# stijnherfst/BrickMap

Hardware: AMD Instinct MI355X
Metric: Mrays/sec (primary x spp x bounces) at 1080p 4-bounce (higher is better)
Workload: dtype f32

## Files before the change

brickmap_amd/_lib.py:

```python
import ctypes as C
import os

_HERE = os.path.dirname(os.path.abspath(__file__))
LIB_PATH = os.path.join(_HERE, "libbrickmap_hip.so")

BM_FLAG_PRIMARY_ONLY = 1
BM_FLAG_SAMPLE_ITEMS = 4
BM_FLAG_COUNTERS = 2
BM_FLAG_ORDERED = 16
BM_FLAG_RAY_DIGEST = 32
BM_QUERY_LOD = 1
BM_QUERY_NO_REQUESTS = 2
BM_VOLUME_ANY = 1
BM_VOXELS_HOST = 0
BM_VOXELS_DEVICE = 1
BRICK_INDEX_BITS = 0x00000FFF
BRICK_LOD_BITS = 0x000FF000
BRICK_REQUESTED_BIT = 0x20000000
BRICK_UNLOADED_BIT = 0x40000000
BRICK_LOADED_BIT = 0x80000000


class BrickmapError(RuntimeError):
    pass
# ... 41 lines not shown

class bm_ray(C.Structure):
    _fields_ = [("origin", C.c_float * 3), ("direction", C.c_float * 3), ("tmax", C.c_float), ("reserved", C.c_uint32)]


class bm_ray_hit(C.Structure):
    _fields_ = [("distance", C.c_float), ("normal", C.c_float * 3), ("voxel", C.c_int32 * 3), ("level", C.c_int32)]


class bm_reproject_params(C.Structure):
    _fields_ = [("width", C.c_int32), ("height", C.c_int32), ("max_history", C.c_float), ("flags", C.c_uint32), ("reserved", C.c_uint32)]


class bm_denoise_params(C.Structure):
    _fields_ = [("width", C.c_int32), ("height", C.c_int32), ("iterations", C.c_int32), ("sigma_l", C.c_float), ("flags", C.c_uint32), ("reserved", C.c_uint32)]


class bm_volume(C.Structure):
    _fields_ = [("shape", C.c_int32), ("lo", C.c_int32 * 3), ("hi", C.c_int32 * 3), ("center", C.c_int32 * 3), ("radius", C.c_int32), ("reserved", C.c_uint32)]


class bm_volume_result(C.Structure):
    _fields_ = [("solid", C.c_uint64), ("lo", C.c_int32 * 3), ("hi", C.c_int32 * 3), ("unresolved", C.c_uint32), ("status", C.c_uint32)]


class bm_scene_info(C.Structure):
    _fields_ = [("grid_size", C.c_int32), ("grid_height", C.c_int32), ("supergrid_xy", C.c_int32),
                ("supergrid_z", C.c_int32), ("supercells", C.c_int32), ("queue_capacity", C.c_int32),
                ("lod_distance_8x8x8", C.c_int32), ("lod_distance_2x2x2", C.c_int32),
                ("generated", C.c_int32), ("on_device", C.c_int32),
                ("total_bricks", C.c_uint64), ("resident_bricks", C.c_uint64),
                ("index_bytes", C.c_uint64), ("brick_bytes", C.c_uint64),
                ("pool_bytes", C.c_uint64), ("cube_field_bytes", C.c_uint64),
                ("arena_growths", C.c_uint64), ("arena_copy_growths", C.c_uint64), ("arena_virtual", C.c_int32), ("failed", C.c_int32),
                ("stream_batches", C.c_uint64), ("stream_host_ns", C.c_uint64), ("escape_bytes", C.c_uint64), ("sun_plane_bytes", C.c_uint64)]


COUNTER_NAMES = ("index_loads", "brick_tests", "byte_tests", "voxel_steps", "extend_rays",
                 "shadow_rays", "requests", "paths")


class bm_counters(C.Structure):
    _fields_ = [(n, C.c_uint64) for n in COUNTER_NAMES]

    def as_dict(self):
        return {n: int(getattr(self, n)) for n in COUNTER_NAMES}


SCHED_NAMES = ("step_runs", "step_lanes", "candidate_runs", "candidate_lanes", "shade_runs", "shade_lanes", "connect_runs", "connect_lanes",
               "step_cycles", "candidate_cycles", "shade_cycles", "drain_cycles", "total_cycles", "jump_runs", "jump_lanes", "waves")


class bm_sched_stats(C.Structure):
    _fields_ = [(n, C.c_uint64) for n in SCHED_NAMES]


_vp, _i, _u32p = C.c_void_p, C.c_int, C.POINTER(C.c_uint32)
SIGNATURES = {
    "bm_last_error_string": (C.c_char_p, []),
    "bm_device_count": (_i, [C.POINTER(C.c_int)]),
    "bm_device_name": (_i, [_i, C.c_char_p, C.c_size_t, C.POINTER(C.c_int)]),
    "bm_scene_create": (_i, [_i, _i, _i, C.POINTER(_vp)]),
    "bm_scene_destroy": (None, [_vp]),
    "bm_scene_set_lod": (_i, [_vp, _i, _i]),
    "bm_scene_set_queue_capacity": (_i, [_vp, _i]),
    "bm_scene_set_streaming_mode": (_i, [_vp, _i]),
    "bm_scene_generate": (_i, [_vp, _i]),
    "bm_scene_generate_supercell": (_i, [_vp, _i, _i, _i]),
    "bm_scene_preload_all": (_i, [_vp]),
    "bm_scene_reset_residency": (_i, [_vp]),
    "bm_scene_process_load_queue": (_i, [_vp, _u32p]),
    "bm_scene_dump": (_i, [_vp, C.c_char_p]),
    "bm_scene_get_info": (_i, [_vp, C.POINTER(bm_scene_info)]),
    "bm_scene_host_supercell": (_i, [_vp, _i, _vp, _u32p, _vp, C.c_uint32]),
    "bm_scene_device_indices": (_i, [_vp, _i, _vp]),
    "bm_scene_device_brick": (_i, [_vp, _i, C.c_uint32, _vp]),
    "bm_scene_column_heights": (_i, [_vp, _i, _i, _vp]),
    "bm_scene_edit": (_i, [_vp, _i, C.POINTER(bm_edit), _vp]),
    "bm_scene_set_voxels": (_i, [_vp, _i, _vp, _vp, _vp]),
    "bm_scene_device_cube_field": (_i, [_vp, _vp, C.c_size_t, C.POINTER(C.c_size_t)]),
    "bm_scene_host_cube_field": (_i, [_vp, _vp, C.c_size_t, C.POINTER(C.c_size_t)]),
    "bm_scene_escape_table": (_i, [_vp, _vp, C.c_size_t, C.POINTER(C.c_size_t)]),
    "bm_scene_sun_plane": (_i, [_vp, _vp, C.c_size_t, C.POINTER(C.c_size_t), _vp]),
    "bm_scene_sun_plane_stats": (_i, [_vp, C.POINTER(C.c_uint64), C.POINTER(C.c_float)]),
    "bm_scene_last_edit_ms": (_i, [_vp, C.POINTER(C.c_float), C.POINTER(C.c_float)]),
    "bm_scene_load_voxels": (_i, [_vp, _vp, C.c_size_t, _i, _vp]),
    "bm_scene_host_voxels": (_i, [_vp, _vp, C.c_size_t, C.POINTER(C.c_size_t)]),
    "bm_scene_last_load_ms": (_i, [_vp, C.POINTER(C.c_float), C.POINTER(C.c_float), C.POINTER(C.c_float)]),
    "bm_scene_write_region": (_i, [_vp, C.POINTER(bm_region), _i, _vp, _i, _vp]),
    "bm_scene_read_region": (_i, [_vp, C.POINTER(bm_region), _vp, _i, _vp]),
    "bm_scene_last_region_ms": (_i, [_vp] + [C.POINTER(C.c_float)] * 4),
    "bm_scene_cast_rays": (_i, [_vp, C.c_int64, _vp, _vp, C.c_uint32, _vp, _vp]),
    "bm_scene_query_volumes": (_i, [_vp, C.c_int64, _vp, _vp, C.c_uint32, _vp]),
    "bm_camera_pixel_rays": (_i, [C.POINTER(bm_camera), _i, _i, C.c_int64, _vp, _vp, _vp]),
    "bm_camera_pixel_rays_device": (_i, [_vp, C.POINTER(bm_camera), _i, _i, _vp, _vp]),
    "bm_denoise_workspace_bytes": (_i, [_i, _i, C.POINTER(C.c_size_t)]),
    "bm_denoise": (_i, [_vp, C.POINTER(bm_denoise_params), _vp, _vp, _vp, _vp, C.c_size_t, _vp]),
    "bm_debug_denoise_times": (_i, [_vp, C.POINTER(bm_denoise_params), _vp, _vp, _vp, _vp, C.c_size_t, _vp, C.POINTER(C.c_float)]),
    "bm_host_denoise": (_i, [C.POINTER(bm_denoise_params), _vp, _vp, _vp]),
    "bm_history_bytes": (_i, [_i, _i, C.POINTER(C.c_size_t)]),
    "bm_reproject": (_i, [_vp, C.POINTER(bm_reproject_params), C.POINTER(bm_camera), C.POINTER(bm_camera), _vp, _vp, _vp, _vp, _vp]),
    "bm_host_reproject": (_i, [C.POINTER(bm_reproject_params), C.POINTER(bm_camera), C.POINTER(bm_camera), _vp, _vp, _vp, _vp]),
    "bm_host_column_heights": (_i, [_i, _i, _i, _i, _vp]),
    "bm_host_generate_supercell": (_i, [_i, _i, _i, _i, _i, _vp, _u32p, _vp, C.c_uint32]),
    "bm_host_edit_supercell": (_i, [_i, _i, _i, _i, _i, _vp, _u32p, _vp, C.c_uint32, _i, C.POINTER(bm_edit)]),
    "bm_host_write_region_supercell": (_i, [_i, _i, _i, _i, _i, _vp, _u32p, _vp, C.c_uint32, C.POINTER(bm_region), _i, _vp]),
    "bm_host_load_supercell": (_i, [_i, _i, _i, _i, _i, _vp, _vp, _vp, _u32p]),
    "bm_host_cube_field": (_i, [_i, _i, _vp, C.c_size_t, C.POINTER(C.c_size_t)]),
    "bm_buffer_alloc": (_i, [_i, C.c_size_t, C.POINTER(_vp)]),
    "bm_buffer_free": (_i, [_i, _vp]),
    "bm_buffer_zero": (_i, [_i, _vp, C.c_size_t, _vp]),
    "bm_buffer_read": (_i, [_i, _vp, _vp, C.c_size_t]),
    "bm_buffer_write": (_i, [_i, _vp, _vp, C.c_size_t]),
    "bm_local_rows": (_i, [C.POINTER(bm_frame_params)]),
    "bm_render_frame": (_i, [_vp, C.POINTER(bm_camera), C.POINTER(bm_frame_params), _vp, _vp, _vp]),
    "bm_render_frames": (_i, [_vp, _i, C.POINTER(bm_camera), C.POINTER(bm_frame_params), C.POINTER(_vp), C.POINTER(_vp), _vp]),
    "bm_frame_plan_of": (_i, [C.POINTER(bm_frame_params), _i, C.POINTER(bm_frame_plan)]),
    "bm_launch_plan_of": (_i, [_i, C.POINTER(bm_camera), C.POINTER(bm_frame_params), _vp, _vp, _i, _i, C.POINTER(bm_launch_plan)]),
    "bm_trace_waves_per_simd": (_i, [_i, _i, _i, _i, C.POINTER(C.c_int)]),
    "bm_tuning_overrides": (_i, [C.c_char_p, C.c_size_t]),
    "bm_resolve": (_i, [_vp, _vp, _vp, C.c_int64, _vp]),
    "bm_synchronize": (_i, [_vp]),
    "bm_last_render_ms": (_i, [_vp, C.POINTER(C.c_float)]),
    "bm_render_times": (_i, [_vp, _vp, _i, C.POINTER(C.c_int)]),
    "bm_counters_read": (_i, [_vp, C.POINTER(bm_counters)]),
    "bm_counters_reset": (_i, [_vp]),
    "bm_sched_stats_read": (_i, [_vp, C.POINTER(bm_sched_stats)]),
    "bm_sched_detail_read": (_i, [_vp, _vp]),
    "bm_wavefront_create": (_i, [_vp, C.c_uint32, C.POINTER(_vp)]),
    "bm_wavefront_destroy": (None, [_vp]),
    "bm_wavefront_reset": (_i, [_vp]),
    "bm_wavefront_frame": (_i, [_vp, C.POINTER(bm_camera), C.POINTER(bm_frame_params), _vp, _vp]),
    "bm_wavefront_stats": (_i, [_vp, _u32p]),
    "bm_wavefront_read_queue": (_i, [_vp, _i, C.c_uint32, C.c_uint32, _vp]),
    "bm_wavefront_times": (_i, [_vp, C.POINTER(C.c_float)]),
    "bm_wavefront_counters_read": (_i, [_vp, _i, C.POINTER(bm_counters)]),
    "bm_wavefront_counters_reset": (_i, [_vp]),
    "bm_wavefront_sched_stats_read": (_i, [_vp, _i, C.POINTER(C.c_uint64)]),
    "bm_comm_unique_id": (_i, [_vp]),
    "bm_comm_create": (_i, [_i, _i, _i, _vp, C.POINTER(_vp)]),
    "bm_comm_destroy": (None, [_vp]),
    "bm_comm_info": (_i, [_vp, C.POINTER(C.c_int), C.POINTER(C.c_int)]),
    "bm_comm_available": (_i, []),
    "bm_debug_division_magic": (_i, [C.c_uint32, C.POINTER(C.c_uint32), C.POINTER(C.c_int)]),
    "bm_gather_frame": (_i, [_vp, _vp, _vp, _i, _i, _i, _i, _vp]),
    "bm_gather_frames": (_i, [_vp, _vp, _vp, _i, _i, _i, _i, _i, _vp]),
    "bm_reduce_frame": (_i, [_vp, _vp, _vp, C.c_int64, _i, _vp]),
    "bm_probe_streams": (_i, [_i, _i, C.POINTER(_vp)]),
    "bm_release_streams": (None, [_i, C.POINTER(_vp)]),
    "bm_comm_barrier": (_i, [_vp, _vp]),
    "bm_comm_selftest": (_i, [_vp, _vp]),
    "bm_debug_assemble_frame": (_i, [_i, _vp, _vp, _vp, _i, _i, _i, _i, _i, _i, _vp]),
    "bm_debug_sincos": (_i, [_i, _i, _vp, _vp, _vp]),
    "bm_debug_sky": (_i, [_i, _vp, _i, _vp, _vp, _vp, _vp]),
}

_lib = None


def load():
    global _lib
    if _lib is not None:
        return _lib
    if not os.path.exists(LIB_PATH):
        raise BrickmapError(
            f"{LIB_PATH} is missing: build it with `python -c 'import __graft_entry__ as g; g.build()'` "
# ... 19 lines not shown
```

brickmap_amd/csrc/capi.cpp:

```cpp
#include <cmath>
#include <cstdint>
#include <cstring>
#include <limits>
#include <string>
#include <vector>
#include <new>

#include "camera_rays.h"
#include "denoise.h"
#include "kernels.h"
#include "reproject.h"
#include "scene.h"
#include "wavefront.h"

struct bm_scene {
	bm::Scene impl;
	explicit bm_scene(int device) : impl(device) {}
};

struct bm_wavefront {
	bm::Wavefront impl;
	bm_wavefront(bm::Scene* scene, uint32_t queue_size) : impl(scene, queue_size) {}
};

// ... 21 lines not shown

int bm_device_name(int device, char* buf, size_t buflen, int* compute_units) {
	hipDeviceProp_t prop;
	BM_HIP(hipGetDeviceProperties(&prop, device));
	if (buf && buflen) {
		std::strncpy(buf, prop.gcnArchName, buflen - 1);
		buf[buflen - 1] = 0;
	}
	if (compute_units) *compute_units = prop.multiProcessorCount;
	return 0;
}

int bm_scene_create(int device, int grid_size, int grid_height, bm_scene** out) {
	if (!out) { set_error("null argument"); return BM_EINVAL; }
	*out = nullptr;
	bm_scene* s = new (std::nothrow) bm_scene(device);
	if (!s) { set_error("out of host memory"); return BM_EINVAL; }
	if (int e = s->impl.init(grid_size, grid_height)) {
		delete s;
		return e;
	}
	*out = s;
	return 0;
}

void bm_scene_destroy(bm_scene* scene) { delete scene; }

int bm_scene_set_lod(bm_scene* scene, int lod8, int lod2) { BM_NEED(scene); return scene->impl.set_lod(lod8, lod2); }
int bm_scene_set_queue_capacity(bm_scene* scene, int capacity) { BM_NEED(scene); return scene->impl.set_queue_capacity(capacity); }
int bm_scene_set_streaming_mode(bm_scene* scene, int overlapped) { BM_NEED(scene); return scene->impl.set_streaming_mode(overlapped); }
int bm_scene_generate(bm_scene* scene, int threads) { BM_NEED(scene); return scene->impl.generate(threads); }
int bm_scene_generate_supercell(bm_scene* scene, int sx, int sy, int sz) { BM_NEED(scene); return scene->impl.generate_supercell(sx, sy, sz); }
int bm_scene_preload_all(bm_scene* scene) { BM_NEED(scene); return scene->impl.preload_all(); }
int bm_scene_reset_residency(bm_scene* scene) { BM_NEED(scene); return scene->impl.reset_residency(); }
int bm_scene_process_load_queue(bm_scene* scene, uint32_t* serviced) { BM_NEED(scene); return scene->impl.process_load_queue(serviced); }
int bm_scene_dump(bm_scene* scene, const char* path) { BM_NEED(scene); return scene->impl.dump(path); }
int bm_scene_get_info(bm_scene* scene, bm_scene_info* info) { BM_NEED(scene); return scene->impl.info(info); }

int bm_scene_host_supercell(bm_scene* scene, int supercell, uint32_t* indices4096, uint32_t* brick_count, uint32_t* bricks, uint32_t brick_capacity) {
	BM_NEED(scene);
	bm::World& w = scene->impl.world;
	if (supercell < 0 || supercell >= static_cast<int>(w.supercells.size())) { set_error("bad supercell (or world not generated)"); return BM_EINVAL; }
	const bm::HostSupercell& c = w.supercells[supercell];
	if (c.indices.size() != static_cast<size_t>(bm::kCellsPerSupercell)) { set_error("supercell not generated"); return BM_ESTATE; }
	if (indices4096) std::memcpy(indices4096, c.indices.data(), bm::kCellsPerSupercell * sizeof(uint32_t));
	if (brick_count) *brick_count = static_cast<uint32_t>(c.bricks.size());
	if (bricks) {
		const size_t n = c.bricks.size() < brick_capacity ? c.bricks.size() : brick_capacity;
		std::memcpy(bricks, c.bricks.data(), n * sizeof(bm::Brick));
	}
	return 0;
}

int bm_scene_device_indices(bm_scene* scene, int supercell, uint32_t* indices4096) { BM_NEED(scene); return scene->impl.device_indices(supercell, indices4096); }

int bm_scene_device_brick(bm_scene* scene, int supercell, uint32_t device_slot, uint32_t* out16) { BM_NEED(scene); return scene->impl.device_brick(supercell, device_slot, out16); }

int bm_scene_edit(bm_scene* scene, int count, const bm_edit* edits, void* hip_stream) {
	BM_NEED(scene);
	return scene->impl.edit(count, edits, static_cast<hipStream_t>(hip_stream));
}

int bm_scene_set_voxels(bm_scene* scene, int n, const int32_t* xyz, const uint8_t* values, void* hip_stream) {
	BM_NEED(scene);
	if (n < 0 || (n > 0 && (!xyz || !values))) { set_error("bm_scene_set_voxels: bad count or null argument"); return BM_EINVAL; }
	std::vector<bm_edit> edits;
	edits.reserve(static_cast<size_t>(n));
	for (int i = 0; i < n; ++i) {
		const int32_t* v = xyz + 3 * static_cast<size_t>(i);
		if (v[0] < 0 || v[1] < 0 || v[2] < 0 || v[0] == INT32_MAX || v[1] == INT32_MAX || v[2] == INT32_MAX) continue;
		bm_edit e{};
		e.op = values[i] ? BM_EDIT_SET : BM_EDIT_CLEAR;
		e.shape = BM_EDIT_BOX;
		for (int k = 0; k < 3; ++k) { e.lo[k] = v[k]; e.hi[k] = v[k] + 1; }
		edits.push_back(e);
	}
	return scene->impl.edit(static_cast<int>(edits.size()), edits.data(), static_cast<hipStream_t>(hip_stream));
}

int bm_scene_device_cube_field(bm_scene* scene, uint8_t* dst, size_t capacity, size_t* bytes) { BM_NEED(scene); return scene->impl.device_cube_field(dst, capacity, bytes); }
int bm_scene_host_cube_field(bm_scene* scene, uint8_t* dst, size_t capacity, size_t* bytes) { BM_NEED(scene); return scene->impl.host_cube_field(dst, capacity, bytes); }
int bm_scene_escape_table(bm_scene* scene, int32_t* dst, size_t capacity, size_t* count) { BM_NEED(scene); return scene->impl.escape_table(dst, capacity, count); }
int bm_scene_sun_plane(bm_scene* scene, uint8_t* dst, size_t capacity, size_t* bytes, int32_t* plan12) { BM_NEED(scene); return scene->impl.sun_plane(dst, capacity, bytes, plan12); }
int bm_scene_sun_plane_stats(bm_scene* scene, uint64_t* builds, float* last_build_ms) { BM_NEED(scene); return scene->impl.sun_plane_stats(builds, last_build_ms); }
int bm_scene_last_edit_ms(bm_scene* scene, float* scatter_ms, float* field_ms) { BM_NEED(scene); return scene->impl.last_edit_ms(scatter_ms, field_ms); }

int bm_scene_load_voxels(bm_scene* scene, const uint8_t* voxels, size_t bytes, int where, void* hip_stream) {
	BM_NEED(scene);
	return scene->impl.load_voxels(voxels, bytes, where, static_cast<hipStream_t>(hip_stream));
}
int bm_scene_host_voxels(bm_scene* scene, uint8_t* dst, size_t capacity, size_t* bytes) { BM_NEED(scene); return scene->impl.host_voxels(dst, capacity, bytes); }
int bm_scene_last_load_ms(bm_scene* scene, float* pack_ms, float* field_ms, float* mirror_ms) { BM_NEED(scene); return scene->impl.last_load_ms(pack_ms, field_ms, mirror_ms); }

int bm_scene_write_region(bm_scene* scene, const bm_region* region, int op, const uint8_t* voxels, int where, void* hip_stream) {
	BM_NEED(scene);
	return scene->impl.write_region(region, op, voxels, where, static_cast<hipStream_t>(hip_stream));
}
int bm_scene_read_region(bm_scene* scene, const bm_region* region, uint8_t* voxels, int where, void* hip_stream) {
	BM_NEED(scene);
	return scene->impl.read_region(region, voxels, where, static_cast<hipStream_t>(hip_stream));
}
int bm_scene_last_region_ms(bm_scene* scene, float* pack_ms, float* copy_ms, float* scatter_ms, float* field_ms) {
	BM_NEED(scene);
	return scene->impl.last_region_ms(pack_ms, copy_ms, scatter_ms, field_ms);
}

int bm_scene_cast_rays(bm_scene* scene, int64_t n, const bm_ray* rays_dev, bm_ray_hit* hits_dev, uint32_t flags, const float lod_origin[3], void* hip_stream) {
	BM_NEED(scene);
	return scene->impl.cast_rays(n, rays_dev, hits_dev, flags, lod_origin, static_cast<hipStream_t>(hip_stream));
}

int bm_scene_query_volumes(bm_scene* scene, int64_t n, const bm_volume* volumes_dev, bm_volume_result* results_dev, uint32_t flags, void* hip_stream) {
	BM_NEED(scene);
	return scene->impl.query_volumes(n, volumes_dev, results_dev, flags, static_cast<hipStream_t>(hip_stream));
}

int bm_camera_pixel_rays(const bm_camera* camera, int width, int height, int64_t n, const float* px, const float* py, bm_ray* out) {
	if (!camera || width <= 0 || height <= 0 || width > 65535 || height > 65535 || n < 0 || (n > 0 && (!px || !py || !out))) {
		set_error("bm_camera_pixel_rays: bad argument");
		return BM_EINVAL;
	}
	bm_frame_params p{};
	p.width = width; p.height = height; p.spp = 1; p.band_rows = height; p.shard_count = 1;
	bm::FrameConstants fc;
	if (int e = bm::fill_frame_constants(camera, &p, &fc)) return e;
	const float W = static_cast<float>(width), H = static_cast<float>(height);
	for (int64_t i = 0; i < n; ++i) {
		bm_ray& r = out[i];
		bm::pixel_ray_direction(fc.dir, fc.right, fc.up, W, H, px[i], py[i], r.direction);
		for (int k = 0; k < 3; ++k) r.origin[k] = fc.origin[k];
		r.tmax = std::numeric_limits<float>::infinity();
		r.reserved = 0;
	}
	return 0;
}

int bm_camera_pixel_rays_device(bm_scene* scene, const bm_camera* camera, int width, int height, bm_ray* rays_dev, void* hip_stream) {
	BM_NEED(scene);
	return scene->impl.pixel_rays(camera, width, height, rays_dev, static_cast<hipStream_t>(hip_stream));
}

int bm_denoise_workspace_bytes(int width, int height, size_t* bytes) {
	if (!bytes || width < 1 || height < 1 || width > 65535 || height > 65535) { set_error("bm_denoise_workspace_bytes: bad argument"); return BM_EINVAL; }
	*bytes = bm::denoise_workspace_bytes(width, height);
	return 0;
}

int bm_denoise(bm_scene* scene, const bm_denoise_params* params, const float* accum_dev, const bm_ray_hit* hits_dev, float* out_dev, void* workspace_dev,
			   size_t workspace_bytes, void* hip_stream) {
	BM_NEED(scene);
	return scene->impl.denoise(params, accum_dev, hits_dev, out_dev, workspace_dev, workspace_bytes, static_cast<hipStream_t>(hip_stream));
}

int bm_debug_denoise_times(bm_scene* scene, const bm_denoise_params* params, const float* accum_dev, const bm_ray_hit* hits_dev, float* out_dev,
						   void* workspace_dev, size_t workspace_bytes, void* hip_stream, float* kernel_ms) {
	BM_NEED(scene);
	if (!kernel_ms) { set_error("bm_debug_denoise_times: null argument"); return BM_EINVAL; }
	return scene->impl.denoise(params, accum_dev, hits_dev, out_dev, workspace_dev, workspace_bytes, static_cast<hipStream_t>(hip_stream), kernel_ms);
}

int bm_history_bytes(int width, int height, size_t* bytes) {
	if (!bytes || width < 1 || height < 1 || width > 65535 || height > 65535) { set_error("bm_history_bytes: bad argument"); return BM_EINVAL; }
	*bytes = bm::history_bytes(width, height);
	return 0;
}

// ... 354 lines not shown
```

brickmap_amd/csrc/kernels.h:

```cpp
#pragma once
#include <hip/hip_runtime.h>

#include "device_types.h"
#include "reproject.h"
#include "sunfield.h"

namespace bm {
template <class K>
int resident_blocks_per_cu(K kernel, int threads = 256) {
	int n = 0;
	const hipError_t e = hipOccupancyMaxActiveBlocksPerMultiprocessor(&n, kernel, threads, 0);
	return e == hipSuccess && n > 0 ? n : 1;
}

constexpr size_t kWorkCounterBytes = 64 * 32 * sizeof(uint32_t);
int trace_blocks_per_cu(bool instrumented, bool xcd_handout, bool helpers, int ring = 0);
void launch_trace(const DeviceScene& sc, const FrameConstants* fc_dev, DeviceCounters* counters, uint32_t* work_counter, bool instrumented, bool xcd_handout, bool helpers,
				  int ring, long long workgroups, int compute_units, int blocks_per_cu_cap, hipStream_t stream);
void launch_upload(const DeviceScene& sc, const uint32_t* bricks_queue, const uint32_t* indices_queue, uint32_t* arena, uint32_t count,
				   hipStream_t stream);
void launch_pool_moves(const PoolMove* moves, uint32_t count, uint32_t* arena, uint32_t* pool_base, hipStream_t stream);
void launch_snapshot_ring(const int* queue, const uint32_t* count, int* host_positions, uint32_t* host_count, uint32_t capacity, hipStream_t stream);
void launch_resolve(const float* accum, float* out, long long n, hipStream_t stream);
void launch_debug_sincos(int n, const float* x, float* s, float* c, hipStream_t stream);
void launch_debug_sky(const FrameConstants& fc, int n, const float* v, float* sun, float* sky, float* sunsky, hipStream_t stream);

struct FieldUpdate {
	int rx0, rx1, ry0, ry1, rz0, rz1;
	int ay0, ay1, bz0, bz1;
	int cells, cells_height, sg_xy, sg_xy2;
	int cf_shift;
	uint32_t cf_pxy, cf_plane;
};
size_t field_update_tmp_bytes(const FieldUpdate& u);
void launch_edit_scatter(const uint32_t* cells, const uint32_t* words, const uint32_t* slots, const uint32_t* bricks, uint32_t count,
						 uint32_t* index_grid, uint32_t* arena, hipStream_t stream);
void launch_field_update(const uint32_t* index_grid, uint8_t* field, uint8_t* tmp, const FieldUpdate& u, hipStream_t stream);

struct EscapeUpdate {
	int x0, x1, y0, y1;
	int cells, cells_height, sg_xy, sg_xy2;
	int cf_shift;
	uint32_t cf_pxy, cf_plane;
};
size_t escape_columns_bytes(int cells);
void launch_escape_update(const uint32_t* index_grid, int32_t* cols, uint32_t* table, const EscapeUpdate& u, hipStream_t stream);

struct SunBuild {
	SunPlan plan;
	int cells, cells_height, sg_xy, sg_xy2;
	int nd, n1, n2;
	int cf_shift;
	uint32_t cf_pxy, cf_plane;
};
size_t sun_build_tmp_bytes(const SunBuild& u);
void launch_sun_build(const uint32_t* index_grid, const int32_t* cols, const uint32_t* escape, uint8_t* field, uint8_t* tmp, const SunBuild& u, hipStream_t stream);

struct LoadDims {
	uint32_t grid_size;
	uint32_t sg_xy, sg_xy2;
	uint32_t supercells;
};
void launch_load_classify(const uint8_t* voxels, uint32_t* index_grid, const LoadDims& d, hipStream_t stream);
void launch_load_number(uint32_t* index_grid, uint32_t* counts, uint32_t* pool_base, uint32_t* total, const LoadDims& d, hipStream_t stream);
void launch_load_pack(const uint8_t* voxels, const uint32_t* index_grid, const uint32_t* pool_base, uint32_t* arena, const LoadDims& d, hipStream_t stream);

struct RegionDims {
	int lo[3], hi[3], org[3];
	int c0[3], nc[3], g0;
	uint32_t sg_xy, sg_xy2;
	int64_t row_pitch, slice_pitch;
};
void launch_region_pack(const uint8_t* voxels, uint32_t* bricks, const RegionDims& d, hipStream_t stream);
void launch_region_unpack(uint8_t* voxels, const uint32_t* index_grid, const uint32_t* pool_base, const uint32_t* arena, const RegionDims& d, hipStream_t stream);
void launch_region_patch(uint8_t* voxels, const int* cells, const uint32_t* bricks, uint32_t count, const RegionDims& d, hipStream_t stream);
void launch_region_zero(uint8_t* voxels, int64_t row_pitch, int64_t slice_pitch, int64_t nx, int64_t ny, int64_t nz, hipStream_t stream);

int query_blocks_per_cu(bool request);
void launch_query(const DeviceScene& sc, const int campos[3], const void* rays, void* hits, uint32_t n, uint32_t* ticket, int resident_blocks,
				  bool request, hipStream_t stream);

int volume_blocks_per_cu(bool any);
size_t volume_tmp_bytes(uint32_t n);
void launch_volume_query(const DeviceScene& sc, const void* volumes, void* results, uint32_t n, bool any, uint64_t* tmp, int resident_blocks, hipStream_t stream);

constexpr int kDenoiseTiledMaxStep = 2;
void launch_denoise(int width, int height, int iterations, float sigma_l, const float* accum, const void* hits, float* out, void* workspace,
					int tiled_max_step, hipStream_t stream, hipEvent_t* marks = nullptr);
struct PixelRayBasis {
	float right[3], up[3], dir[3], origin[3];
	int width, height;
};
void launch_pixel_rays(const PixelRayBasis& basis, void* rays, hipStream_t stream);
struct ReprojectCameras {
	CameraBasis cur;
	RpPrevCamera prev;
	int width, height;
};
void launch_reproject(const ReprojectCameras& cams, float max_history, const float* accum, const void* hits, const void* history_prev, void* history_out,
					  hipStream_t stream);

int wavefront_blocks_per_cu(bool connect, bool instrumented);
void launch_wf_primary(WfState* st, WfRay* work, const FrameConstants* fc_dev, uint32_t queue_size, uint32_t pixels, hipStream_t stream);
void launch_wf_trace(bool connect, const DeviceScene& sc, const FrameConstants* fc_dev, WfState* st, WfRay* work, const WfShadow* shadow, float* accum,
					 DeviceCounters* counters, uint32_t queue_size, int resident_blocks, void* cold_scratch, hipStream_t stream);
void launch_wf_shade(const WfRay* work, WfRay* next, WfShadow* shadow, float* accum, void* block_counts, WfState* st, const FrameConstants* fc_dev,
					 uint32_t queue_size, hipStream_t stream);
}
```

brickmap_amd/csrc/scene.cpp:

```cpp
#include "scene.h"

#include <algorithm>
#include <atomic>
#include <chrono>
#include <climits>
#include <cmath>
#include <cstddef>
#include <cstdio>
#include <cstdlib>
#include <cstring>
#include <fstream>
#include <thread>
#include <unordered_map>

#include "camera_rays.h"
#include "denoise.h"
#include "escape.h"
#include "kernels.h"

namespace bm {

static thread_local std::string g_error;
void set_error(const std::string& msg) { g_error = msg; }
const char* last_error() { return g_error.c_str(); }
// ... 49 lines not shown
	if (!on_device_) { set_error("scene not generated"); return BM_ESTATE; }
	return 0;
}

int Scene::require_not_failed() const {
	if (failed_) { set_error("a streaming batch failed on this scene: call bm_scene_reset_residency / bm_scene_preload_all"); return BM_ESTATE; }
	return 0;
}

int Scene::init(int grid_size, int grid_height) {
	if (!world.dims.set(grid_size, grid_height)) {
		set_error("grid_size and grid_height must be positive multiples of 128 voxels");
		return BM_EINVAL;
	}
	if (world.dims.cells > 1024 || world.dims.cells_height > 1024) {
		set_error("world too large: at most 8192 voxels along an axis (and see the cube-field limit: cubic worlds up to 5760 voxels a side)");
		return BM_EINVAL;
	}
	if (!cube_field_layout(world.dims).fits) {
		set_error("world too large: the octant cube field (8 planes of (cells_h + 2) x (cells + 2) rows padded to a power of two) must stay below 4 GiB -- cubic worlds up to 5760 voxels a side");
		return BM_EINVAL;
	}
	BM_HIP(hipSetDevice(device_));
	if (int e = load_stream_.create(hipStreamNonBlocking)) return e;
	if (int e = kernel_stream_.create(hipStreamNonBlocking)) return e;
	for (int i = 0; i < kTimingRing; ++i) {
		if (int e = ev_start_[i].create()) return e;
		if (int e = ev_stop_[i].create()) return e;
	}
	for (Event* ev : {&ev_upload_, &ev_snapshot_, &ev_edit_, &ev_edit_caller_}) if (int e = ev->create(hipEventDisableTiming)) return e;
	for (Event& ev : ev_edit_time_) if (int e = ev.create()) return e;
	for (int r = 0; r < 2; ++r) {
		if (int e = h_count_[r].alloc(sizeof(uint32_t))) return e;
		if (int e = d_load_count_[r].alloc(sizeof(uint32_t))) return e;
		BM_HIP(hipMemset(d_load_count_[r], 0, sizeof(uint32_t)));
	}
	if (int e = d_counters_.alloc(sizeof(DeviceCounters))) return e;
	BM_HIP(hipMemset(d_counters_, 0, sizeof(DeviceCounters)));
	if (int e = d_work_counter_.alloc(kWorkCounterBytes * kFrameRing)) return e;
	if (int e = d_frame_constants_.alloc(kFrameRing * sizeof(FrameConstants))) return e;
	if (int e = h_frame_constants_.alloc(kFrameRing * sizeof(FrameConstants))) return e;
	std::fill(ring_owner_, ring_owner_ + kFrameRing, -1ll);
	hipDeviceProp_t prop;
	BM_HIP(hipGetDeviceProperties(&prop, device_));
	compute_units_ = prop.multiProcessorCount;
	blocks_per_cu_[0] = blocks_per_cu_[1] = 0;
	if (tuning().blocks_per_cu > 0) blocks_per_cu_[0] = tuning().blocks_per_cu;

	return alloc_queue();
}

int Scene::alloc_queue() {
	BM_HIP(hipSetDevice(device_));
	const size_t n = static_cast<size_t>(queue_cap_);
	for (int r = 0; r < 2; ++r) {
		if (int e = h_positions_[r].alloc(n * 3 * sizeof(int))) return e;
		if (int e = d_load_queue_[r].alloc(n * 3 * sizeof(int))) return e;
		BM_HIP(hipMemset(d_load_queue_[r], 0, n * 3 * sizeof(int)));
		BM_HIP(hipMemset(d_load_count_[r], 0, sizeof(uint32_t)));
	}
	if (int e = h_bricks_.alloc(n * sizeof(Brick))) return e;
	if (int e = h_indices_.alloc(n * sizeof(uint32_t))) return e;
	if (int e = d_bricks_queue_.alloc(n * sizeof(Brick))) return e;
	if (int e = d_indices_queue_.alloc(n * sizeof(uint32_t))) return e;
	if (int e = d_positions_.alloc(n * 3 * sizeof(int))) return e;
	if (int e = h_moves_.alloc(n * sizeof(PoolMove))) return e;
	if (int e = d_moves_.alloc(n * sizeof(PoolMove))) return e;
	use_ring(0);
	snapshot_pending_ = false;
	view_.queue_cap = static_cast<uint32_t>(queue_cap_);
	return 0;
}

void Scene::use_ring(int ring) {
	ring_cur_ = ring;
	view_.load_queue = d_load_queue_[ring];
	view_.load_queue_count = d_load_count_[ring];
}

void Scene::residency_rebuilt(bool preloaded) {
	use_ring(0);
	snapshot_pending_ = false;
	preloaded_ = preloaded;
	staging_busy_ = false;
	failed_ = false;
	stream_batches_ = stream_host_ns_ = 0;
	upload_seq_ = 0;
	for (FrameStream& f : frame_streams_) f.upload_seen = 0;
}

int Scene::set_streaming_mode(int overlapped) {
	BM_HIP(hipSetDevice(device_));
	BM_HIP(hipDeviceSynchronize());
	if (snapshot_pending_) {
		snapshot_pending_ = false;
		const uint32_t count = std::min<uint32_t>(static_cast<uint32_t>(queue_cap_), *h_count_[ring_snapshot_]);
		if (count > 0) {
			if (int e = service_ring(ring_snapshot_, count, nullptr)) return e;
		}
		BM_HIP(hipDeviceSynchronize());
	}
	if (overlapped_ && !overlapped && ring_cur_ != 0) {
		BM_HIP(hipMemcpy(d_load_queue_[0], d_load_queue_[1], static_cast<size_t>(queue_cap_) * 3 * sizeof(int), hipMemcpyDeviceToDevice));
		BM_HIP(hipMemcpy(d_load_count_[0], d_load_count_[1], sizeof(uint32_t), hipMemcpyDeviceToDevice));
		BM_HIP(hipMemset(d_load_count_[1], 0, sizeof(uint32_t)));
		use_ring(0);
	}
	overlapped_ = overlapped != 0;
	return 0;
}

int Scene::set_lod(int lod8, int lod2) {
	lod8_ = lod8;
	lod2_ = lod2;
	view_.lod_distance_8x8x8 = lod8;
	view_.lod_distance_2x2x2 = lod2;
	return 0;
}

int Scene::set_queue_capacity(int cap) {
	if (cap <= 0) { set_error("queue capacity must be positive"); return BM_EINVAL; }
	if (on_device_) { set_error("set the queue capacity before bm_scene_generate"); return BM_ESTATE; }
	BM_HIP(hipSetDevice(device_));
	BM_HIP(hipDeviceSynchronize());
	queue_cap_ = cap;
	return alloc_queue();
}

void Scene::free_device() {
	(void)d_index_grid_.release();
	(void)d_pool_base_.release();
	arena_.close();
	(void)d_cube_field_.release();
	sun_plane_ = sun_built_ = false;
	(void)d_escape_.release();
	(void)d_escape_cols_.release();
	on_device_ = false;
}

int Scene::arena_fit(uint64_t bricks) {
	arena_.reset();
	bool left_unmapped = false;
	const int e = arena_.reserve(std::max<uint64_t>(bricks, 1), true, &left_unmapped);
	if (left_unmapped) failed_ = true;
	view_.brick_arena = arena_.base();
	return e;
}

int Scene::pool_region(uint32_t bricks, uint32_t* offset) {
	const int e = arena_.region_alloc(bricks, offset);
	view_.brick_arena = arena_.base();
	return e;
}

int Scene::allocate_device() {
	BM_HIP(hipSetDevice(device_));
	free_device();
	const WorldDims& d = world.dims;
	uint64_t run = 0;
	for (int i = 0; i < d.supercells; ++i) run += world.supercells[i].bricks.size();
	if (run >= (1ull << 32)) { set_error("world has more than 2^32 bricks"); return BM_EINVAL; }
	if (int e = alloc_index_grid()) return e;
	if (int e = arena_.open(device_, 4 * run + 32ull * static_cast<uint64_t>(d.supercells) + (1ull << 16))) return e;
	view_.brick_arena = arena_.base();
	if (int e = alloc_cube_field()) return e;
	{
		std::vector<uint8_t> field;
		world.build_cube_field(field, 8);
		const int X = d.cells + 2, Z = d.cells_height + 2;
		for (int o = 0; o < 8; ++o)
			BM_HIP(hipMemcpy2D(d_cube_field_ + static_cast<size_t>(o) * view_.cf_plane, static_cast<size_t>(1) << view_.cf_shift, field.data() + static_cast<size_t>(o) * X * X * Z, X, X,
							   static_cast<size_t>(X) * Z, hipMemcpyHostToDevice));
	}
	set_view_dims();
	on_device_ = true;
	if (int e = reset_residency()) return e;
	launch_escape_update(d_index_grid_, d_escape_cols_, d_escape_, escape_update_box(0, d.cells, 0, d.cells), load_stream_);
	BM_HIP(hipGetLastError());
	BM_HIP(hipStreamSynchronize(load_stream_));
	return 0;
}

int Scene::alloc_index_grid() {
	const WorldDims& d = world.dims;
	const size_t index_bytes = static_cast<size_t>(d.supercells) * kCellsPerSupercell * sizeof(uint32_t);
	if (int e = d_index_grid_.alloc(index_bytes)) return e;
	if (int e = d_pool_base_.alloc(static_cast<size_t>(d.supercells) * sizeof(uint32_t))) return e;
	BM_HIP(hipMemset(d_pool_base_, 0, static_cast<size_t>(d.supercells) * sizeof(uint32_t)));
	view_.index_grid = d_index_grid_;
	view_.pool_base = d_pool_base_;
	view_.brick_arena = nullptr;
	return 0;
}

int Scene::alloc_cube_field() {
	const CubeFieldLayout l = cube_field_layout(world.dims);
	if (!l.fits) { set_error("world too large for the 32-bit cube-field offsets of the walk"); return BM_EINVAL; }
	sun_plane_ = false;
	if (l.ninth) {
		if (d_cube_field_.alloc(l.plane * 9) == 0) sun_plane_ = true;
		else { (void)hipGetLastError(); set_error(""); }
	}
	if (!sun_plane_) { if (int e = d_cube_field_.alloc(l.plane * 8)) return e; }
	sun_built_ = false;
	sun_dirty_ = true;
	BM_HIP(hipMemset(d_cube_field_, 255, d_cube_field_.bytes()));
	view_.cf_shift = l.shift;
	view_.cf_pxy = static_cast<uint32_t>(l.pxy);
	view_.cf_plane = static_cast<uint32_t>(l.plane);
	division_magic(view_.cf_pxy, &view_.cf_magic, &view_.cf_magic_shift);
	view_.cube_field = d_cube_field_;
	if (int e = d_escape_.alloc(escape_entries(view_.cf_pxy) * sizeof(uint32_t))) return e;
	BM_HIP(hipMemset(d_escape_, 0, d_escape_.bytes()));
	if (int e = d_escape_cols_.alloc(escape_columns_bytes(world.dims.cells))) return e;
	view_.escape = d_escape_;
	return 0;
}

EscapeUpdate Scene::escape_update_box(int x0, int x1, int y0, int y1) const {
	const WorldDims& d = world.dims;
	EscapeUpdate u{};
	u.x0 = std::max(0, x0); u.x1 = std::min(d.cells, x1); u.y0 = std::max(0, y0); u.y1 = std::min(d.cells, y1);
	if (u.x1 < u.x0) u.x1 = u.x0;
	if (u.y1 < u.y0) u.y1 = u.y0;
	u.cells = d.cells; u.cells_height = d.cells_height;
	u.sg_xy = d.supergrid_xy; u.sg_xy2 = d.supergrid_xy * d.supergrid_xy;
	u.cf_shift = view_.cf_shift; u.cf_pxy = view_.cf_pxy; u.cf_plane = view_.cf_plane;
	return u;
}

void Scene::set_view_dims() {
	const WorldDims& d = world.dims;
	view_.cells = d.cells;
	view_.cells_height = d.cells_height;
	view_.sg_xy = d.supergrid_xy;
	view_.sg_xy2 = d.supergrid_xy * d.supergrid_xy;
	view_.grid_size_f = static_cast<float>(d.grid_size);
	view_.grid_height_f = static_cast<float>(d.grid_height);
	view_.lod_distance_8x8x8 = lod8_;
	view_.lod_distance_2x2x2 = lod2_;
}

int Scene::generate(int threads) {
	world.generate(threads);
	return allocate_device();
}

int Scene::generate_supercell(int sx, int sy, int sz) {
	const WorldDims& d = world.dims;
	if (sx < 0 || sy < 0 || sz < 0 || sx >= d.supergrid_xy || sy >= d.supergrid_xy || sz >= d.supergrid_z) {
		set_error("supercell coordinates out of range");
		return BM_EINVAL;
	}
	if (on_device_) { set_error("bm_scene_generate_supercell: the scene is on the device (call it before bm_scene_generate)"); return BM_ESTATE; }
	world.generate_supercell(sx, sy, sz);
	return 0;
}

int Scene::reset_residency() {
	if (int e = require_on_device()) return e;
	BM_HIP(hipSetDevice(device_));
	BM_HIP(hipDeviceSynchronize());
	const WorldDims& d = world.dims;
	std::vector<uint32_t> words(static_cast<size_t>(d.supercells) * kCellsPerSupercell);
	std::vector<uint32_t> bases(d.supercells, 0u);
	uint64_t initial = 0;
	for (int i = 0; i < d.supercells; ++i) initial += world.supercells[i].bricks.empty() ? 0u : kStartingPool;
	if (int e = arena_fit(initial)) return e;
	for (int i = 0; i < d.supercells; ++i) {
		HostSupercell& c = world.supercells[i];
		c.resident = 0;
		c.pool_capacity = 0;
		c.pool_base = 0;
		c.dev_slot.assign(c.bricks.size(), kNoDeviceSlot);
		c.pool_free.clear();
		if (!c.bricks.empty()) {
			if (int e = pool_region(kStartingPool, &c.pool_base)) return e;
			c.pool_capacity = kStartingPool;
		}
		bases[i] = c.pool_base;
		uint32_t* dst = &words[static_cast<size_t>(i) * kCellsPerSupercell];
		for (int j = 0; j < kCellsPerSupercell; ++j)
			dst[j] = (c.indices[j] & BM_BRICK_LOADED_BIT) ? (BM_BRICK_UNLOADED_BIT | (c.indices[j] & BM_BRICK_LOD_BITS)) : 0u;
	}
	BM_HIP(hipMemcpy(d_index_grid_, words.data(), words.size() * sizeof(uint32_t), hipMemcpyHostToDevice));
	BM_HIP(hipMemcpy(d_pool_base_, bases.data(), bases.size() * sizeof(uint32_t), hipMemcpyHostToDevice));
	for (int r = 0; r < 2; ++r) BM_HIP(hipMemset(d_load_count_[r], 0, sizeof(uint32_t)));
	resident_bricks_ = 0;
	residency_rebuilt(false);
	return 0;
}

int Scene::preload_all() {
	if (int e = require_on_device()) return e;
	BM_HIP(hipSetDevice(device_));
// ... 297 lines not shown
			launch_pool_moves(d_moves_, n_moves, arena_.base(), d_pool_base_, load_stream_);
			BM_HIP(hipGetLastError());
		}
		launch_upload(ring_view, d_bricks_queue_, d_indices_queue_, arena_.base(), kept, load_stream_);
		BM_HIP(hipGetLastError());
		BM_HIP(hipMemsetAsync(d_load_count_[ring], 0, sizeof(uint32_t), load_stream_));
		BM_HIP(hipEventRecord(ev_upload_, load_stream_));
		return 0;
	};
	if (int e = queue()) { failed_ = true; return e; }
	arena_.commit_freed_regions();
	staging_busy_ = true;
	upload_seq_++;
	resident_bricks_ += kept;
	if (serviced) *serviced = kept;
	stream_batches_++;
	stream_host_ns_ += static_cast<uint64_t>(std::chrono::duration_cast<std::chrono::nanoseconds>(std::chrono::steady_clock::now() - t_host0).count());
	return 0;
}

int Scene::process_load_queue(uint32_t* serviced) {
	if (serviced) *serviced = 0;
	if (int e = require_on_device()) return e;
	if (int e = require_not_failed()) return e;
	BM_HIP(hipSetDevice(device_));
	if (!overlapped_) {
		if (int e = wait_frames_on_host()) return e;
		BM_HIP(hipMemcpyAsync(h_count_[0], d_load_count_[0], sizeof(uint32_t), hipMemcpyDeviceToHost, load_stream_));
		BM_HIP(hipStreamSynchronize(load_stream_));
		const uint32_t count = std::min<uint32_t>(static_cast<uint32_t>(queue_cap_), *h_count_[0]);
		if (count == 0) return 0;
		BM_HIP(hipMemcpyAsync(h_positions_[0], d_load_queue_[0], static_cast<size_t>(count) * 3 * sizeof(int), hipMemcpyDeviceToHost, load_stream_));
		BM_HIP(hipStreamSynchronize(load_stream_));
		return service_ring(0, count, serviced);
	}
	if (snapshot_pending_) {
		BM_HIP(hipEventSynchronize(ev_snapshot_));
		snapshot_pending_ = false;
		const uint32_t count = std::min<uint32_t>(static_cast<uint32_t>(queue_cap_), *h_count_[ring_snapshot_]);
		if (count > 0) {
			if (int e = service_ring(ring_snapshot_, count, serviced)) return e;
		}
	}
	if (int e = order_load_stream_behind_frames()) return e;
	const int ring = ring_cur_;
	{
		int* dev_positions = nullptr;
		uint32_t* dev_count = nullptr;
		BM_HIP(hipHostGetDevicePointer(reinterpret_cast<void**>(&dev_positions), h_positions_[ring], 0));
		BM_HIP(hipHostGetDevicePointer(reinterpret_cast<void**>(&dev_count), h_count_[ring], 0));
		launch_snapshot_ring(d_load_queue_[ring], d_load_count_[ring], dev_positions, dev_count, static_cast<uint32_t>(queue_cap_), load_stream_);
		BM_HIP(hipGetLastError());
	}
	BM_HIP(hipEventRecord(ev_snapshot_, load_stream_));
	snapshot_pending_ = true;
	ring_snapshot_ = ring;
	use_ring(ring ^ 1);
	return 0;
}

int Scene::dump(const char* path) {
	std::ofstream file(path ? path : "dump.txt");
	if (!file) { set_error("cannot open dump file"); return BM_EINVAL; }
	for (const auto& c : world.supercells) file << c.resident << "\n";
	return 0;
}

int Scene::info(bm_scene_info* out) {
	if (!out) { set_error("null argument"); return BM_EINVAL; }
	const WorldDims& d = world.dims;
	std::memset(out, 0, sizeof *out);
	out->grid_size = d.grid_size; out->grid_height = d.grid_height;
	out->supergrid_xy = d.supergrid_xy; out->supergrid_z = d.supergrid_z; out->supercells = d.supercells;
	out->queue_capacity = queue_cap_;
	out->lod_distance_8x8x8 = lod8_; out->lod_distance_2x2x2 = lod2_;
	out->generated = world.generated ? 1 : 0;
	out->on_device = on_device_ ? 1 : 0;
	out->total_bricks = world.generated ? world.total_bricks() : 0;
	out->resident_bricks = resident_bricks_;
	out->index_bytes = on_device_ ? static_cast<uint64_t>(d.supercells) * kCellsPerSupercell * 4 : 0;
	out->brick_bytes = on_device_ ? arena_.capacity() * 64 : 0;
	out->pool_bytes = on_device_ ? arena_.pool_bricks() * 64 : 0;
	out->cube_field_bytes = on_device_ ? 8 * static_cast<uint64_t>(view_.cf_plane) : 0;
	out->escape_bytes = on_device_ ? d_escape_.bytes() : 0;
	out->sun_plane_bytes = on_device_ && sun_plane_ ? static_cast<uint64_t>(view_.cf_plane) + d_sun_tmp_.bytes() : 0;
	out->arena_growths = arena_.growths();
	out->arena_copy_growths = arena_.copy_growths();
	out->arena_virtual = arena_.is_virtual() ? 1 : 0;
	out->failed = failed_ ? 1 : 0;
	out->stream_batches = stream_batches_;
	out->stream_host_ns = stream_host_ns_;
	return 0;
}

int Scene::device_indices(int supercell, uint32_t* out4096) {
	if (int e = require_on_device()) return e;
	if (supercell < 0 || supercell >= world.dims.supercells || !out4096) { set_error("bad supercell"); return BM_EINVAL; }
	BM_HIP(hipSetDevice(device_));
	BM_HIP(hipDeviceSynchronize());
	BM_HIP(hipMemcpy(out4096, d_index_grid_ + static_cast<size_t>(supercell) * kCellsPerSupercell, kCellsPerSupercell * 4, hipMemcpyDeviceToHost));
	return 0;
}

int Scene::device_brick(int supercell, uint32_t device_slot, uint32_t* out16) {
	if (int e = require_on_device()) return e;
	if (supercell < 0 || supercell >= world.dims.supercells || !out16 || device_slot >= world.supercells[supercell].resident) {
		set_error("bad supercell or slot");
		return BM_EINVAL;
	}
	BM_HIP(hipSetDevice(device_));
	BM_HIP(hipDeviceSynchronize());
	BM_HIP(hipMemcpy(out16, arena_.base() + (static_cast<size_t>(world.supercells[supercell].pool_base) + device_slot) * kBrickWords, sizeof(Brick), hipMemcpyDeviceToHost));
	return 0;
}

int Scene::edit(int count, const bm_edit* edits, hipStream_t stream) {
	std::string why;
	if (!World::validate_edits(edits, count, &why)) { set_error("bm_scene_edit: " + why); return BM_EINVAL; }
	if (!on_device_) { set_error("bm_scene_edit: scene not generated"); return BM_ESTATE; }
	if (int e = require_not_failed()) return e;
	const WorldDims& d = world.dims;
	std::vector<int> reached;
	{
		std::vector<uint8_t> seen(static_cast<size_t>(d.supercells), 0);
		for (int i = 0; i < count; ++i) {
			int lo[3], hi[3];
			if (!World::edit_bounds(d, edits[i], lo, hi)) continue;
			for (int sz = lo[2] / kColumnSpan; sz <= (hi[2] - 1) / kColumnSpan; ++sz)
				for (int sy = lo[1] / kColumnSpan; sy <= (hi[1] - 1) / kColumnSpan; ++sy)
					for (int sx = lo[0] / kColumnSpan; sx <= (hi[0] - 1) / kColumnSpan; ++sx) {
						const int sc = d.supercell_id(sx, sy, sz);
						if (!seen[sc]) { seen[sc] = 1; reached.push_back(sc); }
					}
		}
	}
	if (reached.empty()) return 0;
	std::sort(reached.begin(), reached.end());
	BM_HIP(hipSetDevice(device_));
	if (int e = wait_edit_staging()) return e;

	DeviceBatch batch;
	std::vector<uint32_t> old_words;
	std::vector<uint8_t> touched;
	for (const int sci : reached) {
		HostSupercell& c = world.supercells[sci];
		const int sx = sci % d.supergrid_xy, sy = (sci / d.supergrid_xy) % d.supergrid_xy, sz = sci / (d.supergrid_xy * d.supergrid_xy);
		old_words = c.indices;
		touched.assign(kCellsPerSupercell, 0);
		World::edit_supercell(d, c, sx, sy, sz, edits, count, touched.data());
		if (int e = stage_touched(sci, old_words, touched.data(), batch)) return e;
	}
	bool scattered = false, field = false;
	if (int e = submit_batch(batch, stream, ev_edit_time_, &scattered, &field)) return e;
	if (scattered) {
		edit_timed_ = true;
		edit_field_timed_ = field;
	}
	return 0;
}

int Scene::wait_edit_staging() {
	if (edit_busy_) { BM_HIP(hipEventSynchronize(ev_edit_)); edit_busy_ = false; }
	return 0;
}

int Scene::stage_touched(int sci, const std::vector<uint32_t>& old_words, const uint8_t* touched, DeviceBatch& b) {
	const WorldDims& d = world.dims;
	HostSupercell& c = world.supercells[sci];
	const int sx = sci % d.supergrid_xy, sy = (sci / d.supergrid_xy) % d.supergrid_xy, sz = sci / (d.supergrid_xy * d.supergrid_xy);
	const std::vector<uint16_t>& old_dev = c.dev_slot;
	std::vector<uint16_t> dev(c.bricks.size(), kNoDeviceSlot);
	for (int j = 0; j < kCellsPerSupercell; ++j)
		if (c.indices[j] && !touched[j]) dev[c.indices[j] & BM_BRICK_INDEX_BITS] = old_dev[c.indices[j] & BM_BRICK_INDEX_BITS];
	std::vector<int> fresh_cells;
	for (int j = 0; j < kCellsPerSupercell; ++j) {
		if (!touched[j]) continue;
		const uint32_t ow = old_words[j], nw = c.indices[j];
		const uint16_t ods = ow ? old_dev[ow & BM_BRICK_INDEX_BITS] : kNoDeviceSlot;
		if (ods != kNoDeviceSlot) {
			if (nw) dev[nw & BM_BRICK_INDEX_BITS] = ods;
			else { c.pool_free.push_back(ods); resident_bricks_--; }
		} else if (nw && preloaded_) {
			fresh_cells.push_back(j);
		}
		if ((ow != 0) != (nw != 0)) {
			const int g[3] = {sx * kSupercell + (j & 15), sy * kSupercell + ((j >> 4) & 15), sz * kSupercell + (j >> 8)};
			for (int k = 0; k < 3; ++k) { b.box_lo[k] = std::min(b.box_lo[k], g[k]); b.box_hi[k] = std::max(b.box_hi[k], g[k]); }
		}
	}
	if (!fresh_cells.empty()) {
		const uint32_t reuse = static_cast<uint32_t>(std::min(fresh_cells.size(), c.pool_free.size()));
		const uint32_t appends = static_cast<uint32_t>(fresh_cells.size()) - reuse;
		if (c.resident + appends > c.pool_capacity) {
			uint32_t grown = kStartingPool;
			while (grown < c.resident + appends || grown < 2 * c.pool_capacity) grown *= 2;
			uint32_t fresh = 0;
			if (int e = pool_region(grown, &fresh)) { failed_ = true; return e; }
			b.moves.push_back(PoolMove{c.pool_capacity ? c.pool_base : fresh, fresh, c.pool_capacity ? c.resident : 0u, static_cast<uint32_t>(sci)});
			if (c.pool_capacity > 0) arena_.region_free_deferred(c.pool_capacity, c.pool_base);
			c.pool_base = fresh;
			c.pool_capacity = grown;
		}
		for (const int j : fresh_cells) {
			uint32_t ds;
			if (!c.pool_free.empty()) { ds = c.pool_free.back(); c.pool_free.pop_back(); }
			else ds = c.resident++;
			dev[c.indices[j] & BM_BRICK_INDEX_BITS] = static_cast<uint16_t>(ds);
			resident_bricks_++;
		}
	}
	c.dev_slot.swap(dev);
	for (int j = 0; j < kCellsPerSupercell; ++j) {
		if (!touched[j]) continue;
		const uint32_t nw = c.indices[j];
		const uint16_t ds = nw ? c.dev_slot[nw & BM_BRICK_INDEX_BITS] : kNoDeviceSlot;
		b.cells.push_back(static_cast<uint32_t>(sci) * kCellsPerSupercell + static_cast<uint32_t>(j));
		if (!nw) b.words.push_back(0u);
		else if (ds == kNoDeviceSlot) b.words.push_back(BM_BRICK_UNLOADED_BIT | (nw & BM_BRICK_LOD_BITS));
		else b.words.push_back(ds | BM_BRICK_LOADED_BIT | (nw & BM_BRICK_LOD_BITS));
		b.slots.push_back(ds == kNoDeviceSlot ? 0xFFFFFFFFu : c.pool_base + ds);
		b.bricks.push_back(nw ? c.bricks[nw & BM_BRICK_INDEX_BITS] : Brick{});
	}
	return 0;
}

int Scene::submit_batch(DeviceBatch& b, hipStream_t stream, Event* times, bool* scattered, bool* field_updated) {
	const WorldDims& d = world.dims;
	*scattered = *field_updated = false;
	const uint32_t n = static_cast<uint32_t>(b.cells.size());
	if (n == 0) {
		arena_.commit_freed_regions();
		return 0;
	}

	auto up = [](size_t v) { return (v + 63) / 64 * 64; };
	const size_t o_cells = up(b.moves.size() * sizeof(PoolMove)), o_words = o_cells + up(n * 4ull), o_slots = o_words + up(n * 4ull),
				 o_bricks = o_slots + up(n * 4ull), bytes = o_bricks + n * sizeof(Brick);
	const bool field = b.box_hi[0] >= 0;
	const FieldUpdate fu = field ? field_update_box(d, b.box_lo, b.box_hi) : FieldUpdate{};
	auto queue = [&]() -> int {
		if (bytes > d_edit_.bytes()) {
			BM_HIP(hipStreamSynchronize(load_stream_));
			const size_t cap = std::max<size_t>(bytes * 2, 1 << 16);
			if (int e = h_edit_.reserve(cap)) return e;
			if (int e = d_edit_.reserve(cap)) return e;
		}
		if (field && field_update_tmp_bytes(fu) > d_cf_tmp_.bytes()) {
			BM_HIP(hipStreamSynchronize(load_stream_));
			if (int e = d_cf_tmp_.reserve(field_update_tmp_bytes(fu))) return e;
		}
		if (!b.moves.empty()) std::memcpy(h_edit_, b.moves.data(), b.moves.size() * sizeof(PoolMove));
		std::memcpy(h_edit_ + o_cells, b.cells.data(), n * 4ull);
		std::memcpy(h_edit_ + o_words, b.words.data(), n * 4ull);
		std::memcpy(h_edit_ + o_slots, b.slots.data(), n * 4ull);
		std::memcpy(h_edit_ + o_bricks, b.bricks.data(), n * sizeof(Brick));
		if (int e = order_load_stream_behind_frames()) return e;
		BM_HIP(hipEventRecord(ev_edit_caller_, stream));
		BM_HIP(hipStreamWaitEvent(load_stream_, ev_edit_caller_, 0));
		BM_HIP(hipMemcpyAsync(d_edit_, h_edit_, bytes, hipMemcpyHostToDevice, load_stream_));
		BM_HIP(hipEventRecord(ev_edit_, load_stream_));
		BM_HIP(hipEventRecord(times[0], load_stream_));
		if (!b.moves.empty()) {
			launch_pool_moves(reinterpret_cast<const PoolMove*>(d_edit_.get()), static_cast<uint32_t>(b.moves.size()), arena_.base(), d_pool_base_, load_stream_);
			BM_HIP(hipGetLastError());
		}
		launch_edit_scatter(reinterpret_cast<const uint32_t*>(d_edit_ + o_cells), reinterpret_cast<const uint32_t*>(d_edit_ + o_words),
							reinterpret_cast<const uint32_t*>(d_edit_ + o_slots), reinterpret_cast<const uint32_t*>(d_edit_ + o_bricks), n, d_index_grid_, arena_.base(),
							load_stream_);
		BM_HIP(hipGetLastError());
		BM_HIP(hipEventRecord(times[1], load_stream_));
		if (field) {
			launch_field_update(d_index_grid_, d_cube_field_, d_cf_tmp_, fu, load_stream_);
			BM_HIP(hipGetLastError());
			launch_escape_update(d_index_grid_, d_escape_cols_, d_escape_, escape_update_box(b.box_lo[0], b.box_hi[0] + 1, b.box_lo[1], b.box_hi[1] + 1), load_stream_);
			BM_HIP(hipGetLastError());
			sun_dirty_ = true;
		}
		BM_HIP(hipEventRecord(times[2], load_stream_));
		BM_HIP(hipEventRecord(ev_upload_, load_stream_));
		return 0;
	};
	if (int e = queue()) { failed_ = true; return e; }
	arena_.commit_freed_regions();
	edit_busy_ = true;
	upload_seq_++;
	*scattered = true;
	*field_updated = field;
	return 0;
}

int Scene::last_edit_ms(float* scatter_ms, float* field_ms) {
	if (!scatter_ms || !field_ms) { set_error("null argument"); return BM_EINVAL; }
	if (!edit_timed_) { set_error("no edit has changed the scene yet"); return BM_ESTATE; }
	BM_HIP(hipSetDevice(device_));
	BM_HIP(hipEventSynchronize(ev_edit_time_[2]));
	BM_HIP(hipEventElapsedTime(scatter_ms, ev_edit_time_[0], ev_edit_time_[1]));
	BM_HIP(hipEventElapsedTime(field_ms, ev_edit_time_[1], ev_edit_time_[2]));
	if (!edit_field_timed_) *field_ms = 0.0f;
	return 0;
}

namespace {
template <class F> void for_outside_slabs(const int32_t blo[3], const int32_t bhi[3], bool inside, const int lo[3], const int hi[3], F f) {
	if (!inside) { f(blo[0], bhi[0], blo[1], bhi[1], blo[2], bhi[2]); return; }
	if (blo[2] < lo[2]) f(blo[0], bhi[0], blo[1], bhi[1], blo[2], lo[2]);
	if (hi[2] < bhi[2]) f(blo[0], bhi[0], blo[1], bhi[1], hi[2], bhi[2]);
	if (blo[1] < lo[1]) f(blo[0], bhi[0], blo[1], lo[1], lo[2], hi[2]);
	if (hi[1] < bhi[1]) f(blo[0], bhi[0], hi[1], bhi[1], lo[2], hi[2]);
	if (blo[0] < lo[0]) f(blo[0], lo[0], lo[1], hi[1], lo[2], hi[2]);
	if (hi[0] < bhi[0]) f(hi[0], bhi[0], lo[1], hi[1], lo[2], hi[2]);
}
int64_t region_offset(const bm_region& r, int64_t x, int64_t y, int64_t z) { return (z - r.lo[2]) * r.slice_pitch + (y - r.lo[1]) * r.row_pitch + (x - r.lo[0]); }
}

int Scene::check_region(const char* who, const bm_region* region, const void* voxels, int where, bm_region* r, uint64_t* span) {
	const std::string at = std::string(who) + ": ";
	if (!region || !voxels) { set_error(at + "null region or volume"); return BM_EINVAL; }
	*r = *region;
	std::string why;
	if (!World::validate_region(r, &why, span)) { set_error(at + why); return BM_EINVAL; }
	if (where != BM_VOXELS_HOST && where != BM_VOXELS_DEVICE) { set_error(at + "`where` is BM_VOXELS_HOST or BM_VOXELS_DEVICE"); return BM_EINVAL; }
	if (!on_device_) { set_error(at + "scene not generated"); return BM_ESTATE; }
	if (int e = require_not_failed()) return e;
	BM_HIP(hipSetDevice(device_));
	if (where == BM_VOXELS_DEVICE && *span > 0 && !device_span_ok(static_cast<const uint8_t*>(voxels), *span)) {
		set_error(at + "BM_VOXELS_DEVICE needs the volume's whole span inside one allocation of the scene's device");
		return BM_EINVAL;
	}
	return 0;
}

RegionDims Scene::region_dims(const bm_region& r, const int lo[3], const int hi[3]) const {
	RegionDims rd{};
	for (int k = 0; k < 3; ++k) {
		rd.lo[k] = lo[k]; rd.hi[k] = hi[k]; rd.org[k] = r.lo[k];
		rd.c0[k] = lo[k] >> 3;
		rd.nc[k] = ((hi[k] - 1) >> 3) - rd.c0[k] + 1;
	}
	rd.g0 = rd.c0[0] >> 4;
	rd.sg_xy = static_cast<uint32_t>(world.dims.supergrid_xy);
	rd.sg_xy2 = rd.sg_xy * rd.sg_xy;
	rd.row_pitch = r.row_pitch;
	rd.slice_pitch = r.slice_pitch;
	return rd;
}

int Scene::write_region(const bm_region* region, int op, const uint8_t* voxels, int where, hipStream_t stream) {
	bm_region r;
	uint64_t span = 0;
	if (op != BM_REGION_REPLACE && op != BM_EDIT_SET && op != BM_EDIT_CLEAR) { set_error("bm_scene_write_region: unknown op"); return BM_EINVAL; }
	if (int e = check_region("bm_scene_write_region", region, voxels, where, &r, &span)) return e;
	const WorldDims& d = world.dims;
	int lo[3], hi[3];
// ... 89 lines not shown
		});
		if (inside) world.store_region(lo, hi, r.lo, voxels, r.row_pitch, r.slice_pitch, 16);
		return 0;
	}
	std::vector<int> cells;
	std::vector<Brick> bricks;
	if (inside && !preloaded_)
		for (int cz = lo[2] >> 3; cz <= (hi[2] - 1) >> 3; ++cz)
			for (int cy = lo[1] >> 3; cy <= (hi[1] - 1) >> 3; ++cy)
				for (int cx = lo[0] >> 3; cx <= (hi[0] - 1) >> 3; ++cx) {
					const HostSupercell& c = world.supercells[d.supercell_id(cx / kSupercell, cy / kSupercell, cz / kSupercell)];
					const uint32_t word = c.indices[cell_local_index(cx, cy, cz)];
					if (word == 0 || c.dev_slot[word & BM_BRICK_INDEX_BITS] != kNoDeviceSlot) continue;
					cells.insert(cells.end(), {cx, cy, cz});
					bricks.push_back(c.bricks[word & BM_BRICK_INDEX_BITS]);
				}
	const size_t n = bricks.size(), o_bricks = (n * 3 * sizeof(int) + 63) / 64 * 64, bytes = o_bricks + n * sizeof(Brick);
	if (n > 0) {
		if (int e = ev_region_read_.create(hipEventDisableTiming)) return e;
		if (region_read_busy_) { BM_HIP(hipEventSynchronize(ev_region_read_)); region_read_busy_ = false; }
		if (int e = h_patch_.reserve(std::max<size_t>(bytes, 1 << 16))) return e;
		if (int e = d_patch_.reserve(std::max<size_t>(bytes, 1 << 16))) return e;
		std::memcpy(h_patch_, cells.data(), n * 3 * sizeof(int));
		std::memcpy(h_patch_ + o_bricks, bricks.data(), n * sizeof(Brick));
	}
	DeviceScene view;
	if (int e = begin_frame(stream, &view, nullptr)) return e;
	for_outside_slabs(r.lo, r.hi, inside, lo, hi, [&](int64_t x0, int64_t x1, int64_t y0, int64_t y1, int64_t z0, int64_t z1) {
		launch_region_zero(voxels + region_offset(r, x0, y0, z0), r.row_pitch, r.slice_pitch, x1 - x0, y1 - y0, z1 - z0, stream);
	});
	if (inside) {
		const RegionDims rd = region_dims(r, lo, hi);
		launch_region_unpack(voxels, view.index_grid, view.pool_base, view.brick_arena, rd, stream);
		if (n > 0) {
			BM_HIP(hipMemcpyAsync(d_patch_, h_patch_, bytes, hipMemcpyHostToDevice, stream));
			launch_region_patch(voxels, reinterpret_cast<const int*>(d_patch_.get()), reinterpret_cast<const uint32_t*>(d_patch_ + o_bricks), static_cast<uint32_t>(n), rd, stream);
			BM_HIP(hipEventRecord(ev_region_read_, stream));
			region_read_busy_ = true;
		}
	}
	BM_HIP(hipGetLastError());
	end_frame(stream);
	return 0;
}

int Scene::device_cube_field(uint8_t* dst, size_t capacity, size_t* bytes) {
	if (int e = require_on_device()) return e;
	const WorldDims& d = world.dims;
	const size_t X = static_cast<size_t>(d.cells) + 2, Z = static_cast<size_t>(d.cells_height) + 2, need = 8 * X * X * Z;
	if (bytes) *bytes = need;
	if (!dst) return 0;
	if (capacity < need) { set_error("cube field buffer too small"); return BM_EINVAL; }
	BM_HIP(hipSetDevice(device_));
	BM_HIP(hipDeviceSynchronize());
	BM_HIP(hipMemcpy2D(dst, X, d_cube_field_, static_cast<size_t>(1) << view_.cf_shift, X, 8 * X * Z, hipMemcpyDeviceToHost));
	return 0;
}

int Scene::escape_table(int32_t* dst, size_t capacity, size_t* count) {
	if (int e = require_on_device()) return e;
	const WorldDims& d = world.dims;
	const size_t plane = static_cast<size_t>(d.cells) * d.cells, need = 8 * plane;
	if (count) *count = need;
	if (!dst) return 0;
	if (capacity < need) { set_error("escape table buffer too small"); return BM_EINVAL; }
	BM_HIP(hipSetDevice(device_));
	BM_HIP(hipDeviceSynchronize());
	std::vector<uint32_t> entries(escape_entries(view_.cf_pxy));
	BM_HIP(hipMemcpy(entries.data(), d_escape_, entries.size() * sizeof(uint32_t), hipMemcpyDeviceToHost));
	for (int o = 0; o < 8; ++o)
		for (int y = 0; y < d.cells; ++y)
			for (int x = 0; x < d.cells; ++x)
				dst[o * plane + static_cast<size_t>(y) * d.cells + x] = escape_height_of(o, entries[escape_index(o, view_.cf_shift, view_.cf_pxy, x, y)], view_.cf_pxy, view_.cf_plane);
	return 0;
}

int Scene::ensure_sun_plane(const FrameConstants& fc, bool* usable) {
	*usable = false;
	if (!sun_plane_) return 0;
	const SunPlan plan = sun_plan(fc.cone_dir, fc.cone_extent);
	if (!plan.valid) return 0;
	const float key[4] = {fc.cone_dir[0], fc.cone_dir[1], fc.cone_dir[2], fc.cone_extent};
	*usable = true;
	if (sun_built_ && !sun_dirty_ && std::memcmp(key, sun_key_, sizeof key) == 0) return 0;
	const WorldDims& d = world.dims;
	const int n[3] = {d.cells, d.cells, d.cells_height};
	SunBuild u{};
	u.plan = plan;
	u.cells = d.cells; u.cells_height = d.cells_height;
	u.sg_xy = d.supergrid_xy; u.sg_xy2 = d.supergrid_xy * d.supergrid_xy;
	u.nd = n[plan.dom]; u.n1 = n[plan.m1]; u.n2 = n[plan.m2];
	u.cf_shift = view_.cf_shift; u.cf_pxy = view_.cf_pxy; u.cf_plane = view_.cf_plane;
	*usable = false;
	for (Event& ev : ev_sun_time_) if (int e = ev.create()) return e;
	if (sun_build_tmp_bytes(u) > d_sun_tmp_.bytes()) {
		BM_HIP(hipStreamSynchronize(load_stream_));
		if (d_sun_tmp_.reserve(sun_build_tmp_bytes(u)) != 0) { (void)hipGetLastError(); set_error(""); return 0; }
	}
	if (int e = order_load_stream_behind_frames()) return e;
	BM_HIP(hipEventRecord(ev_sun_time_[0], load_stream_));
	launch_sun_build(d_index_grid_, d_escape_cols_, d_escape_, d_cube_field_, d_sun_tmp_, u, load_stream_);
	BM_HIP(hipGetLastError());
	BM_HIP(hipEventRecord(ev_sun_time_[1], load_stream_));
	BM_HIP(hipEventRecord(ev_upload_, load_stream_));
	upload_seq_++;
	std::memcpy(sun_key_, key, sizeof key);
	sun_plan_ = plan;
	sun_built_ = true;
	sun_dirty_ = false;
	sun_builds_++;
	*usable = true;
	return 0;
}

int Scene::sun_plane(uint8_t* dst, size_t capacity, size_t* bytes, int32_t* plan12) {
	if (int e = require_on_device()) return e;
	const WorldDims& d = world.dims;
	const bool have = sun_plane_ && sun_built_;
	const size_t X = static_cast<size_t>(d.cells) + 2, Z = static_cast<size_t>(d.cells_height) + 2, need = have ? X * X * Z : 0;
	if (bytes) *bytes = need;
	if (plan12) {
		const SunPlan p = have ? sun_plan_ : SunPlan{};
		const int32_t v[12] = {p.valid, p.octant, p.dom, p.m1, p.m2, p.lo1, p.hi1, p.lo2, p.hi2, p.clear, p.rise, kSunBins};
		std::memcpy(plan12, v, sizeof v);
	}
	if (!dst || !have) return 0;
	if (capacity < need) { set_error("sun plane buffer too small"); return BM_EINVAL; }
	BM_HIP(hipSetDevice(device_));
	BM_HIP(hipDeviceSynchronize());
	BM_HIP(hipMemcpy2D(dst, X, d_cube_field_ + 8 * static_cast<size_t>(view_.cf_plane), static_cast<size_t>(1) << view_.cf_shift, X, X * Z, hipMemcpyDeviceToHost));
	return 0;
}

int Scene::sun_plane_stats(uint64_t* builds, float* last_build_ms) {
	if (!builds || !last_build_ms) { set_error("null argument"); return BM_EINVAL; }
	*builds = sun_builds_;
	*last_build_ms = 0.0f;
	if (sun_builds_ == 0) return 0;
	BM_HIP(hipSetDevice(device_));
	BM_HIP(hipEventSynchronize(ev_sun_time_[1]));
	BM_HIP(hipEventElapsedTime(last_build_ms, ev_sun_time_[0], ev_sun_time_[1]));
	return 0;
}

int Scene::host_cube_field(uint8_t* dst, size_t capacity, size_t* bytes) {
	const WorldDims& d = world.dims;
	const size_t X = static_cast<size_t>(d.cells) + 2, Z = static_cast<size_t>(d.cells_height) + 2, need = 8 * X * X * Z;
	if (bytes) *bytes = need;
	if (!dst) return 0;
	if (!world.generated) { set_error("world not generated"); return BM_ESTATE; }
	if (capacity < need) { set_error("cube field buffer too small"); return BM_EINVAL; }
	std::vector<uint8_t> f;
	world.build_cube_field(f, 8);
	std::memcpy(dst, f.data(), need);
	return 0;
}

int Scene::render(const bm_camera* cam, const bm_frame_params* fp, float* accum, uint32_t* dbg, hipStream_t stream) {
	return render_frames(1, cam, fp, &accum, dbg ? &dbg : nullptr, stream);
}

int Scene::render_frames(int count, const bm_camera* cams, const bm_frame_params* fps, float* const* accums, uint32_t* const* dbgs, hipStream_t stream) {
	if (int e = require_on_device()) return e;
	LaunchPlan plan;
	if (int e = plan_launch(count, cams, fps, accums, dbgs, world.dims.cells, world.dims.cells_height, &plan)) return e;
	std::vector<FrameConstants>& fcs = plan.frames;
	const FrameConstants& fc = fcs[0];
	BM_HIP(hipSetDevice(device_));
	if (!plan.instrumented && !(fc.flags & BM_FLAG_PRIMARY_ONLY) && fc.spp >= 1) {
		bool usable = false;
		if (int e = ensure_sun_plane(fc, &usable)) return e;
		if (usable)
			for (FrameConstants& f : fcs)
				if (std::memcmp(f.cone_dir, sun_key_, 3 * sizeof(float)) == 0 && f.cone_extent == sun_key_[3]) f.shadow_field_off = 8u * view_.cf_plane;
	}
	if (int e = frame_begin(stream)) return e;
	const int slot = static_cast<int>(launches_ % kTimingRing);
	if (launches_ >= kTimingRing) BM_HIP(hipEventSynchronize(ev_stop_[slot]));
	int first = ring_next_;
	if (first + count > kFrameRing) first = 0;
	long long waited = -1;
	for (int e = first; e < first + count; ++e) {
		const long long owner = ring_owner_[e];
		if (owner >= 0 && owner != waited && launches_ - owner < kTimingRing) {
			BM_HIP(hipEventSynchronize(ev_stop_[owner % kTimingRing]));
			waited = owner;
		}
	}
	uint32_t* const work_counter = d_work_counter_ + static_cast<size_t>(first) * (kWorkCounterBytes / sizeof(uint32_t));
#ifdef BM_PHASE_TIMING
	DeviceCounters* const counters = d_counters_;
#else
	DeviceCounters* const counters = (fc.flags & BM_FLAG_COUNTERS) ? d_counters_.get() : nullptr;
#endif
	auto enqueue = [&]() -> int {
		BM_HIP(hipMemsetAsync(work_counter, 0, kWorkCounterBytes * static_cast<size_t>(plan.counter_blocks), stream));
		std::memcpy(h_frame_constants_ + first, fcs.data(), sizeof(FrameConstants) * static_cast<size_t>(count));
		BM_HIP(hipMemcpyAsync(d_frame_constants_ + first, h_frame_constants_ + first, sizeof(FrameConstants) * static_cast<size_t>(count), hipMemcpyHostToDevice, stream));
		BM_HIP(hipEventRecord(ev_start_[slot], stream));
		launch_trace(view_, d_frame_constants_ + first, counters, work_counter, plan.instrumented, fc.xcd_handout != 0, fc.helpers != 0, plan.ring_mode, plan.workgroups,
					 compute_units_, blocks_per_cu_[plan.instrumented ? 1 : 0], stream);
		BM_HIP(hipGetLastError());
		BM_HIP(hipEventRecord(ev_stop_[slot], stream));
		return frame_end(stream);
	};
	if (int e = enqueue()) {
		(void)hipStreamSynchronize(stream);
		return e;
	}
	for (int e = first; e < first + count; ++e) ring_owner_[e] = launches_;
	ring_next_ = first + count;
	launches_++;
	return 0;
// ... 239 lines not shown
```

brickmap_amd/csrc/scene.h:

```cpp
#pragma once
#include <hip/hip_runtime.h>

#include <string>
#include <vector>

#include "../../include/brickmap.h"
#include "arena.h"
#include "device_types.h"
#include "error.h"
#include "frame_plan.h"
#include "hip_owned.h"
#include "kernels.h"
#include "world.h"

namespace bm {

class Scene {
public:
	explicit Scene(int device) : device_(device) {}
	~Scene();

	int init(int grid_size, int grid_height);
	int set_lod(int lod8, int lod2);
	int set_queue_capacity(int cap);
	int set_streaming_mode(int overlapped);
	int generate(int threads);
	int generate_supercell(int sx, int sy, int sz);
	int preload_all();
	int reset_residency();
	int process_load_queue(uint32_t* serviced);
	int dump(const char* path);
	int info(bm_scene_info* out);
	int device_indices(int supercell, uint32_t* out4096);
	int device_brick(int supercell, uint32_t device_slot, uint32_t* out16);
	int edit(int count, const bm_edit* edits, hipStream_t stream);
	int device_cube_field(uint8_t* dst, size_t capacity, size_t* bytes);
	int host_cube_field(uint8_t* dst, size_t capacity, size_t* bytes);
	int escape_table(int32_t* dst, size_t capacity, size_t* count);
	int last_edit_ms(float* scatter_ms, float* field_ms);
	int sun_plane(uint8_t* dst, size_t capacity, size_t* bytes, int32_t* plan12);
	int sun_plane_stats(uint64_t* builds, float* last_build_ms);
	int write_region(const bm_region* region, int op, const uint8_t* voxels, int where, hipStream_t stream);
	int read_region(const bm_region* region, uint8_t* voxels, int where, hipStream_t stream);
	int last_region_ms(float* pack_ms, float* copy_ms, float* scatter_ms, float* field_ms);
	int load_voxels(const uint8_t* voxels, size_t bytes, int where, hipStream_t stream);
	int host_voxels(uint8_t* dst, size_t capacity, size_t* bytes);
	int last_load_ms(float* pack_ms, float* field_ms, float* mirror_ms);
	int cast_rays(int64_t n, const bm_ray* rays, bm_ray_hit* hits, uint32_t flags, const float* lod_origin, hipStream_t stream);
	int query_volumes(int64_t n, const bm_volume* volumes, bm_volume_result* results, uint32_t flags, hipStream_t stream);
	int render(const bm_camera* cam, const bm_frame_params* fp, float* accum, uint32_t* dbg, hipStream_t stream);
	int render_frames(int count, const bm_camera* cams, const bm_frame_params* fps, float* const* accums, uint32_t* const* dbgs, hipStream_t stream);
	int resolve(const float* accum, float* out, long long n, hipStream_t stream);
	int denoise(const bm_denoise_params* params, const float* accum, const bm_ray_hit* hits, float* out, void* workspace, size_t workspace_bytes, hipStream_t stream,
				float* kernel_ms = nullptr);
	int pixel_rays(const bm_camera* cam, int width, int height, bm_ray* rays, hipStream_t stream);
	int reproject(const bm_reproject_params* params, const bm_camera* cam, const bm_camera* cam_prev, const float* accum, const bm_ray_hit* hits, const void* history_prev,
				  void* history_out, hipStream_t stream);
	int synchronize();
	int last_render_ms(float* ms);
	int render_times(float* ms, int capacity, int* count);
	int counters_read(bm_counters* out);
	int counters_reset();
	int sched_stats_read(bm_sched_stats* out);
	int sched_detail_read(uint64_t* out8);

	int begin_frame(hipStream_t stream, DeviceScene* view, DeviceCounters** counters);
	void end_frame(hipStream_t stream);
	int compute_units() const { return compute_units_; }

	World world;
	int device() const { return device_; }

private:
	int allocate_device();
	int alloc_index_grid();
	int alloc_cube_field();
	int ensure_sun_plane(const FrameConstants& fc, bool* usable);
	EscapeUpdate escape_update_box(int x0, int x1, int y0, int y1) const;
	void set_view_dims();
	int load_voxels_device(const uint8_t* voxels, hipStream_t stream);
	bool device_span_ok(const uint8_t* p, size_t bytes) const;
	struct DeviceBatch {
		std::vector<uint32_t> cells, words, slots;
		std::vector<Brick> bricks;
		std::vector<PoolMove> moves;
		int box_lo[3] = {1 << 30, 1 << 30, 1 << 30}, box_hi[3] = {-1, -1, -1};
	};
	int wait_edit_staging();
	int stage_touched(int sci, const std::vector<uint32_t>& old_words, const uint8_t* touched, DeviceBatch& b);
	int submit_batch(DeviceBatch& b, hipStream_t stream, Event* times, bool* scattered, bool* field_updated);
	int check_region(const char* who, const bm_region* region, const void* voxels, int where, bm_region* r, uint64_t* span);
	RegionDims region_dims(const bm_region& r, const int lo[3], const int hi[3]) const;
	void free_device();
	int alloc_queue();
	int service_ring(int ring, uint32_t count, uint32_t* serviced);
	int require_on_device() const;
	int require_not_failed() const;
	void use_ring(int ring);
	void residency_rebuilt(bool preloaded);
	int arena_fit(uint64_t bricks);
	int pool_region(uint32_t bricks, uint32_t* offset);

	int device_;
	bool on_device_ = false;
	Stream load_stream_, kernel_stream_;
	static constexpr int kTimingRing = 256;
	Event ev_start_[kTimingRing], ev_stop_[kTimingRing];
	Event ev_upload_;
	long long launches_ = 0;
	long long other_frames_ = 0;
	struct FrameStream {
		hipStream_t stream = nullptr;
		Event done;
		uint64_t upload_seen = 0;
		uint64_t last_use = 0;
	};
	static constexpr size_t kMaxFrameStreams = 16;
	std::vector<FrameStream> frame_streams_;
	uint64_t upload_seq_ = 0, frame_seq_ = 0;
	bool staging_busy_ = false;
	bool failed_ = false;
	int frame_begin(hipStream_t stream);
	int frame_end(hipStream_t stream);
	int wait_frames_on_host();
	int order_load_stream_behind_frames();

	DeviceBuffer<uint32_t> d_index_grid_, d_pool_base_;
	DeviceBuffer<uint8_t> d_cube_field_;
	DeviceBuffer<uint32_t> d_escape_;
	DeviceBuffer<int32_t> d_escape_cols_;
	bool sun_plane_ = false, sun_built_ = false, sun_dirty_ = true;
	float sun_key_[4] = {0.f, 0.f, 0.f, 0.f};
	SunPlan sun_plan_{};
	uint64_t sun_builds_ = 0;
	DeviceBuffer<uint8_t> d_sun_tmp_;
	Event ev_sun_time_[2];
	DeviceBuffer<int> d_load_queue_[2];
	DeviceBuffer<uint32_t> d_load_count_[2];
	DeviceBuffer<uint32_t> d_bricks_queue_, d_indices_queue_;
	DeviceBuffer<DeviceCounters> d_counters_;
	static constexpr int kFrameRing = 1024;
	DeviceBuffer<FrameConstants> d_frame_constants_;
	PinnedBuffer<FrameConstants> h_frame_constants_;
	DeviceBuffer<uint32_t> d_work_counter_;
	long long ring_owner_[kFrameRing];
	int ring_next_ = 0;
	int compute_units_ = 0, blocks_per_cu_[2] = {0, 0};
	PinnedBuffer<int> h_positions_[2];
	PinnedBuffer<uint32_t> h_bricks_, h_indices_;
	PinnedBuffer<uint32_t> h_count_[2];
	bool overlapped_ = false, snapshot_pending_ = false;
	int ring_cur_ = 0, ring_snapshot_ = 0;
	Event ev_snapshot_;

	BrickArena arena_;
	static constexpr uint32_t kStartingPool = BrickArena::kStartingPool;
	uint64_t stream_batches_ = 0, stream_host_ns_ = 0;
	PinnedBuffer<PoolMove> h_moves_;
	DeviceBuffer<PoolMove> d_moves_;
	uint64_t resident_bricks_ = 0;
	bool preloaded_ = false;
	DeviceBuffer<int> d_positions_;
	PinnedBuffer<char> h_edit_;
	DeviceBuffer<char> d_edit_;
	Event ev_edit_, ev_edit_caller_;
	Event ev_edit_time_[3];
	bool edit_timed_ = false, edit_field_timed_ = false;
	bool edit_busy_ = false;
	DeviceBuffer<uint8_t> d_cf_tmp_;
	DeviceBuffer<char> d_region_, d_patch_;
	PinnedBuffer<Brick> h_region_;
	PinnedBuffer<char> h_patch_;
	Event ev_region_time_[6], ev_region_read_;
	bool region_timed_ = false, region_packed_ = false, region_scattered_ = false, region_field_ = false, region_read_busy_ = false;
	Event ev_load_time_[6];
	bool load_timed_ = false;
	static constexpr int kQueryRing = 64;
	DeviceBuffer<uint32_t> d_query_tickets_;
	Event ev_query_[kQueryRing];
	uint64_t queries_ = 0;
	int query_blocks_per_cu_[2] = {0, 0};
	DeviceBuffer<uint64_t> d_volume_tmp_;
	Event ev_volume_;
	bool volume_busy_ = false;
	int volume_blocks_per_cu_[2] = {0, 0};
	int queue_cap_ = 1024;
	int lod8_ = 600000, lod2_ = 100000;
	DeviceScene view_{};
};

}
```

brickmap_amd/csrc/sunfield.hip:

```cpp
#include <hip/hip_runtime.h>

#include "escape.h"
#include "global_mem.h"
#include "kernels.h"
#include "sunfield.h"

namespace bm {
namespace {

static_assert(kSunBins == 4, "sixteen lanes per cell: the fold below and the split of the leaving bins");

struct SunTmp {
	int32_t* stamped;
	int32_t* clear[2];
	uint8_t* face[2];
};
__host__ __device__ inline SunTmp sun_tmp(uint8_t* tmp, const SunBuild& u) {
	const size_t n1 = static_cast<size_t>(u.n1), n2 = static_cast<size_t>(u.n2);
	SunTmp t;
	t.stamped = reinterpret_cast<int32_t*>(tmp);
	t.clear[0] = t.stamped + static_cast<size_t>(u.cells) * u.cells;
	t.clear[1] = t.clear[0] + n1 * kSunBins;
	t.face[0] = reinterpret_cast<uint8_t*>(t.clear[1] + n1 * kSunBins);
	t.face[1] = t.face[0] + n1 * n2 * kSunBins * kSunBins;
	return t;
}

__device__ __forceinline__ void sun_cell(const SunBuild& u, int ud, int v1, int v2, int& x, int& y, int& z) {
	const SunPlan& p = u.plan;
	const int cd = sun_coord(p, p.dom, u.nd, ud), c1 = sun_coord(p, p.m1, u.n1, v1), c2 = sun_coord(p, p.m2, u.n2, v2);
	x = p.dom == 0 ? cd : c1;
	y = p.dom == 1 ? cd : (p.dom == 0 ? c1 : c2);
	z = p.dom == 2 ? cd : c2;
}

__device__ __forceinline__ int quadrant_threshold(const uint32_t* escape, const SunBuild& u, int x, int y) {
	return escape_height_of(u.plan.octant, ld32(escape, escape_index(u.plan.octant, u.cf_shift, u.cf_pxy, x, y)), u.cf_pxy, u.cf_plane);
}

__global__ void sun_stamp_quadrant(const uint32_t* __restrict__ escape, int32_t* __restrict__ stamped, const SunBuild u) {
	const uint32_t t = blockIdx.x * blockDim.x + threadIdx.x;
	if (t >= static_cast<uint32_t>(u.cells) * static_cast<uint32_t>(u.cells)) return;
	const int x = static_cast<int>(t % static_cast<uint32_t>(u.cells)), y = static_cast<int>(t / static_cast<uint32_t>(u.cells));
	((g_i32*)stamped)[t] = sun_first_stamped(1 << 20, quadrant_threshold(escape, u, x, y));
}

__global__ void sun_clear_slab(const int32_t* __restrict__ cols, const uint32_t* __restrict__ escape, int32_t* __restrict__ stamped, const int32_t* __restrict__ cn,
							   int32_t* __restrict__ cc, const SunBuild u, const int ud) {
	const SunPlan& p = u.plan;
	const int n1 = u.n1;
	const uint32_t t = blockIdx.x * blockDim.x + threadIdx.x;
	if (t >= static_cast<uint32_t>(n1) * kSunBins) return;
	const int w = static_cast<int>(t / kSunBins), b = static_cast<int>(t % kSunBins);
	auto column = [&](int ww, int& x, int& y) { int z; sun_cell(u, ud, ww, 0, x, y, z); };
	auto height = [&](int ww) {
		if (ww >= n1) return 0;
		int x, y; column(ww, x, y);
		return (ldi32(cols, static_cast<size_t>(y) * u.cells + x) + 1) * kSunHeightUnit;
	};
	auto next = [&](int ww, int bb) { return ww < n1 ? ldi32(cn, static_cast<size_t>(ww) * kSunBins + bb) : 0; };
	((g_i32*)cc)[t] = sun_clear_face_value(p, w, b, height, next);
	if (b == 0) {
		int x, y; column(w, x, y);
		((g_i32*)stamped)[static_cast<size_t>(y) * u.cells + x] = sun_first_stamped(sun_clear_cell(p, w, height, next), quadrant_threshold(escape, u, x, y));
	}
}

__global__ void sun_field_slab(const uint32_t* __restrict__ index_grid, const int32_t* __restrict__ stamped, const uint8_t* __restrict__ fn, uint8_t* __restrict__ fc,
							   uint8_t* __restrict__ field, const SunBuild u, const int ud) {
	const SunPlan& p = u.plan;
	const int n1 = u.n1, n2 = u.n2;
	const uint32_t total = static_cast<uint32_t>(n1) * static_cast<uint32_t>(n2) * (kSunBins * kSunBins);
	const uint32_t t = blockIdx.x * blockDim.x + threadIdx.x;
	const bool live = t < total;
	const uint32_t cell = (live ? t : 0u) / (kSunBins * kSunBins);
	const int b1 = static_cast<int>(t % kSunBins), b2 = static_cast<int>(t / kSunBins % kSunBins);
	const int u1 = static_cast<int>(cell % static_cast<uint32_t>(n1)), u2 = static_cast<int>(cell / static_cast<uint32_t>(n1));
	auto blocked = [&](int v1, int v2) {
		if (v1 >= n1 || v2 >= n2) return true;
		int x, y, z; sun_cell(u, ud, v1, v2, x, y, z);
		return ld32(index_grid, index_word_at(u.sg_xy, u.sg_xy2, x, y, z)) != 0u;
	};
	auto next = [&](int v1, int v2, int g1, int g2) {
		return v1 < n1 && v2 < n2 ? static_cast<int>(ld8(fn, ((static_cast<size_t>(v2) * n1 + v1) * kSunBins + g2) * kSunBins + g1)) : 0;
	};
	if (live) st8(fc, t, static_cast<uint32_t>(sun_face_value(p, u1, u2, b1, b2, blocked, next)));
	const int last1 = kSunBins - 1 + p.hi1, last2 = kSunBins - 1 + p.hi2;
	int part = 254;
	if (live && 2 * b1 <= last1 && 2 * b2 <= last2)
		part = sun_slab_value(u1, u2, 2 * b1, 2 * b1 + 1 < last1 ? 2 * b1 + 1 : last1, 2 * b2, 2 * b2 + 1 < last2 ? 2 * b2 + 1 : last2, [](int, int) { return false; }, next);
	for (int off = 1; off < kSunBins * kSunBins; off <<= 1) { const int o = __shfl_xor(part, off, 64); part = o < part ? o : part; }
	if (live && b1 == 0 && b2 == 0) {
		int x, y, z; sun_cell(u, ud, u1, u2, x, y, z);
		const bool rect = blocked(u1 + 1, u2) || blocked(u1, u2 + 1) || blocked(u1 + 1, u2 + 1);
		uint32_t v = rect ? 1u : static_cast<uint32_t>(part);
		v = z >= ldi32(stamped, static_cast<size_t>(y) * u.cells + x) ? 255u : v;
		v = blocked(u1, u2) ? 0u : v;
		st8(field, 8ull * u.cf_plane + static_cast<size_t>(z + 1) * u.cf_pxy + (static_cast<size_t>(y + 1) << u.cf_shift) + static_cast<size_t>(x + 1), v);
	}
}

}

size_t sun_build_tmp_bytes(const SunBuild& u) {
	const size_t n1 = static_cast<size_t>(u.n1), n2 = static_cast<size_t>(u.n2);
	return (static_cast<size_t>(u.cells) * u.cells + 2 * n1 * kSunBins) * sizeof(int32_t) + 2 * n1 * n2 * kSunBins * kSunBins;
}

void launch_sun_build(const uint32_t* index_grid, const int32_t* cols, const uint32_t* escape, uint8_t* field, uint8_t* tmp, const SunBuild& u, hipStream_t stream) {
	const SunPlan& p = u.plan;
	const SunTmp t = sun_tmp(tmp, u);
	const int nd = u.nd;
	const uint32_t columns = static_cast<uint32_t>(u.cells) * static_cast<uint32_t>(u.cells), clear_lanes = static_cast<uint32_t>(u.n1) * kSunBins;
	const size_t face_bytes = static_cast<size_t>(t.face[1] - t.face[0]);
	const uint32_t face_lanes = static_cast<uint32_t>(face_bytes);
	(void)hipMemsetAsync(t.clear[0], 0, clear_lanes * sizeof(int32_t), stream);
	(void)hipMemsetAsync(t.face[0], 0, face_bytes, stream);
	if (!p.clear) hipLaunchKernelGGL(sun_stamp_quadrant, dim3((columns + 63) / 64), dim3(64), 0, stream, escape, t.stamped, u);
	for (int ud = nd - 1, k = 0; ud >= 0; --ud, k ^= 1) {
		if (p.clear) hipLaunchKernelGGL(sun_clear_slab, dim3((clear_lanes + 63) / 64), dim3(64), 0, stream, cols, escape, t.stamped, t.clear[k], t.clear[k ^ 1], u, ud);
		hipLaunchKernelGGL(sun_field_slab, dim3((face_lanes + 255) / 256), dim3(256), 0, stream, index_grid, t.stamped, t.face[k], t.face[k ^ 1], field, u, ud);
	}
}

}
```

brickmap_amd/csrc/trace.hip:

```cpp
#include <type_traits>

#include "kernels.h"
#include "traverse.h"

namespace bm {

__device__ __forceinline__ uint32_t div_const(uint32_t n, uint32_t magic, int shift) { return magic ? (__umulhi(n, magic) >> shift) : n; }

typedef float bm_v4f __attribute__((ext_vector_type(4)));
typedef __attribute__((address_space(1))) bm_v4f v4f_in_global_memory;
typedef __attribute__((address_space(1))) uint32_t u32_in_global_memory;
__device__ __forceinline__ float4 pixel_load(const float4* p) { const bm_v4f v = *(const v4f_in_global_memory*)p; return make_float4(v.x, v.y, v.z, v.w); }
__device__ __forceinline__ void pixel_store(float4* p, float4 v) { const bm_v4f w = {v.x, v.y, v.z, v.w}; *(v4f_in_global_memory*)p = w; }
__device__ __forceinline__ void record_atomic_add(uint32_t* p, uint32_t v) { (void)__hip_atomic_fetch_add((u32_in_global_memory*)p, v, __ATOMIC_RELAXED, __HIP_MEMORY_SCOPE_AGENT); }

__device__ __forceinline__ void pixel_atomic_add(float* p, float v) {
	typedef __attribute__((address_space(1))) float float_in_global_memory;
	[[clang::atomic(ignore_denormal_mode)]] { (void)__hip_atomic_fetch_add((float_in_global_memory*)p, v, __ATOMIC_RELAXED, __HIP_MEMORY_SCOPE_AGENT); }
}

enum : int { P_GEN = 0, P_EXT_DONE = 1, P_SHD_DONE = 2, P_BOUNCE = 3, P_HELPER = 6 };
enum : int { ST_IDLE = 4, ST_CONN = 5 };

#ifndef BM_WAVES_PER_SIMD
#define BM_WAVES_PER_SIMD 7
#endif
#ifndef BM_ITEM_LANES
#define BM_ITEM_LANES 1
#endif
#ifndef BM_PRIO
#define BM_PRIO 1
#endif
#ifndef BM_PRIO_A
#define BM_PRIO_A 1
#endif
#ifndef BM_PRIO_B
#define BM_PRIO_B 2
#endif
#ifndef BM_PRIO_C
#define BM_PRIO_C 0
#endif
#ifndef BM_WORK_COUNTERS
#define BM_WORK_COUNTERS 16
#endif
#ifndef BM_QUORUM_NUM
#define BM_QUORUM_NUM 1
#endif
#ifndef BM_QUORUM_SHADE_NUM
#define BM_QUORUM_SHADE_NUM 1
#endif
#ifndef BM_QUORUM_DIV
#define BM_QUORUM_DIV 2
#endif
#ifndef BM_QUORUM_SHADE_DIV
#define BM_QUORUM_SHADE_DIV 4
#endif
#ifndef BM_ESCAPE
#define BM_ESCAPE 1
#endif
#ifndef BM_ESCAPE_XCD
#define BM_ESCAPE_XCD 1
#endif
#ifndef BM_STEPS_PER_ROUND
#define BM_STEPS_PER_ROUND 4
#endif
#ifdef BM_ISA_MARKERS
#define BM_REGION(name) asm volatile("; BM_REGION " name)
#else
#define BM_REGION(name) do { } while (0)
#endif
#ifdef BM_PHASE_TIMING
#define BM_TIMED true
#else
#define BM_TIMED DBG
#endif
template <bool DBG, bool XCD = false, bool HELP = false, int RING = 0>
__global__ __launch_bounds__(256, DBG ? 2 : BM_WAVES_PER_SIMD) void trace_paths(const DeviceScene sc, const FrameConstants* __restrict__ fcp,
												  DeviceCounters* __restrict__ counters, uint32_t* __restrict__ work_counter) {
	const FrameConstants& fg = *fcp;
	int ring_pos = 0;
	constexpr bool kRing = RING != 0, kUniform = RING == 2;
#define fc (fcp[RING == 1 ? ring_pos : 0])
	auto more_frames = [&]() { return kUniform ? ring_pos < fg.ring_groups_after : fc.frames_after > 0; };
	float4* accum = reinterpret_cast<float4*>(fc.accum);
	uint32_t* dbg = DBG ? fc.dbg : nullptr;
	__shared__ unsigned long long lds_brick[8 * 256];
	const int lane = threadIdx.x & 63;
	const uint32_t W = static_cast<uint32_t>(fg.width), H = static_cast<uint32_t>(fg.height);
	const uint32_t total_chunks = static_cast<uint32_t>(fg.tiles_x) * static_cast<uint32_t>(fg.tiles_y) * 16u;
	const bool sample_items = (fg.flags & 4u) != 0u;
	constexpr uint32_t kParts = 16u / BM_ITEM_LANES;
	const uint32_t items_per_chunk = (sample_items ? static_cast<uint32_t>(fg.spp > 0 ? fg.spp : 1) : 1u) * (kUniform ? static_cast<uint32_t>(fg.ring_group) : 1u) * kParts;
	const bool atomic_acc = HELP || sample_items;

	uint32_t xy = 0;
	uint32_t p = 0;
	uint32_t local_pixel = 0;
	Tally tally;
	HitInfo info;
	uint32_t d0 = 0, d1 = 0, d2 = 0xFFFFFFFFu, d3 = 0, hseg = 2166136261u, hsh = 2166136261u, next = 0, nsh = 0, loads0 = 0;
	const bool ray_digest = DBG && (fg.flags & 32u) != 0u;
	uint32_t ray_key = 0, ray_loads0 = 0;

	RayState r;
	constexpr bool kEscape = BM_ESCAPE != 0 && !DBG && (BM_ESCAPE_XCD != 0 || !XCD);
	constexpr bool kSun = BM_SUNFIELD != 0 && kEscape && (BM_SUNFIELD_XCD != 0 || !XCD);
	uint32_t esc = 0;
	r.hit = false;
	r.n = mk(0.f, 0.f, 0.f);
	int state = ST_IDLE;
	int pstate = P_GEN;
	int s = 0;
	int s_end = 0;
	int bounces = 0;
	bool shadow = false;
	bool terminated = false;
	f3 hitp = mk(0.f, 0.f, 0.f);
	f3 pn = mk(0.f, 0.f, 0.f);
	f3 scolor = mk(0.f, 0.f, 0.f);
	f3 bdir = mk(0.f, 0.f, 0.f);
	float4 acc = make_float4(0.f, 0.f, 0.f, 0.f);
	auto add_rgb = [&](f3 c) {
		if (HELP) { float* a = reinterpret_cast<float*>(accum + local_pixel); pixel_atomic_add(a + 0, c.x); pixel_atomic_add(a + 1, c.y); pixel_atomic_add(a + 2, c.z); }
		else { acc.x += c.x; acc.y += c.y; acc.z += c.z; }
	};
	auto add_terminated = [&]() {
		if (HELP) pixel_atomic_add(reinterpret_cast<float*>(accum + local_pixel) + 3, 1.f);
		else acc.w += 1.f;
	};

	typename std::conditional<RING == 1, int, bool>::type work_left = 1;
	constexpr uint32_t kCounters = XCD ? 8u : BM_WORK_COUNTERS, kCounterStride = 32;
	constexpr uint32_t kXcdTiles = 16u, kStChunks = kXcdTiles * kXcdTiles * 16u;
	constexpr bool xcd_handout = XCD;
	auto first_counter = [&]() {
		return xcd_handout ? static_cast<int>(blockIdx.x % kCounters)
						   : static_cast<int>((blockIdx.x * 4u + static_cast<uint32_t>(__builtin_amdgcn_readfirstlane(static_cast<int>(threadIdx.x >> 6)))) % kCounters);
	};
	int my_counter = first_counter();
	int counters_done = 0;
	auto round_budget = [&]() {
		const long long budget = (static_cast<long long>(total_chunks) + 64) * (static_cast<long long>(fg.spp) + 1) * (fg.max_bounces + 2) *
								 (2ll * sc.cells + sc.cells_height + 64) * (kRing ? fg.frames_after + 1 : 1);
		return static_cast<long long>((static_cast<unsigned long long>(static_cast<uint32_t>(__builtin_amdgcn_readfirstlane(static_cast<int>(budget >> 32)))) << 32) |
									  static_cast<uint32_t>(__builtin_amdgcn_readfirstlane(static_cast<int>(budget))));
	};
	long long rounds_left = round_budget();
	uint32_t runsA = 0, lanesA = 0, runsB = 0, lanesB = 0, runsC = 0, lanesC = 0, runsD = 0, lanesD = 0, runsJ = 0, lanesJ = 0;

	unsigned long long cycA = 0, cycB = 0, cycC = 0, cycD = 0;
	unsigned long long det[8] = {0, 0, 0, 0, 0, 0, 0, 0};
#ifdef BM_PHASE_TIMING
#define BM_MARK(k, tprev) do { const unsigned long long bm_now_ = __builtin_amdgcn_s_memtime(); det[k] += bm_now_ - tprev; tprev = bm_now_; } while (0)
#else
#define BM_MARK(k, tprev) do { } while (0)
#endif
	const unsigned long long t_begin = BM_TIMED ? __builtin_amdgcn_s_memtime() : 0ull;
	unsigned long long t_dry = 0ull;

	for (;;) {
		BM_REGION("refill");
		const unsigned long long idle = __ballot(state == ST_IDLE);
		const int nI = __popcll(idle);
		if (RING == 1 && work_left == 2 && nI == 64) {
			++ring_pos;
			accum = reinterpret_cast<float4*>(fc.accum);
			if (DBG) dbg = fc.dbg;
			work_left = 1;
		}
		if (work_left == 1 && nI >= fg.refill_min) {
			const int want = nI / BM_ITEM_LANES;
			uint32_t base = 0;
			if (lane == 0) base = atomicAdd(work_counter + (kRing ? static_cast<uint32_t>(ring_pos) * static_cast<uint32_t>(kWorkCounterBytes / sizeof(uint32_t)) : 0u) + my_counter * kCounterStride, static_cast<uint32_t>(want));
			base = __builtin_amdgcn_readfirstlane(base);
			const uint32_t st_x = (static_cast<uint32_t>(fg.tiles_x) + kXcdTiles - 1u) / kXcdTiles, st_y = (static_cast<uint32_t>(fg.tiles_y) + kXcdTiles - 1u) / kXcdTiles;
			const uint32_t total_units = xcd_handout ? st_x * st_y : (total_chunks + 3u) >> 2;
			const uint32_t my_units = total_units > static_cast<uint32_t>(my_counter)
										  ? (total_units - static_cast<uint32_t>(my_counter) + kCounters - 1u) / kCounters : 0u;
			const uint32_t my_tickets = my_units * (xcd_handout ? kStChunks : 4u) * items_per_chunk;
			const uint32_t counter_now = static_cast<uint32_t>(my_counter);
			const int ring_at_refill = kRing ? ring_pos : 0;
			if (kRing && !XCD && base + want >= my_tickets && more_frames()) {
				if (kUniform) ++ring_pos;
				else work_left = 2;
			} else if (base + want >= my_tickets) {
				my_counter = (my_counter + 1) % static_cast<int>(kCounters);
				if (++counters_done >= static_cast<int>(kCounters)) {
					if (kRing && more_frames()) {
						counters_done = 0;
// ... 230 lines not shown
			}
			BM_REGION("C.hand-over");
			if (HELP) {
				const unsigned long long hand_m = __ballot(hand), free_m = __ballot(state == ST_IDLE);
				if (hand_m != 0ull && free_m != 0ull) {
					const int n_pairs = min(__popcll(hand_m), __popcll(free_m));
					const int hrank = __builtin_amdgcn_mbcnt_hi(static_cast<uint32_t>(hand_m >> 32), __builtin_amdgcn_mbcnt_lo(static_cast<uint32_t>(hand_m), 0u));
					const int frank = __builtin_amdgcn_mbcnt_hi(static_cast<uint32_t>(free_m >> 32), __builtin_amdgcn_mbcnt_lo(static_cast<uint32_t>(free_m), 0u));
					const bool gives = hand && hrank < n_pairs, takes = state == ST_IDLE && frank < n_pairs;
					if (gives) {
						const uint32_t k = static_cast<uint32_t>(hrank);
						staging_word(lds_brick, k, 0) = ro.x; staging_word(lds_brick, k, 1) = ro.y; staging_word(lds_brick, k, 2) = ro.z;
						staging_word(lds_brick, k, 3) = rd.x; staging_word(lds_brick, k, 4) = rd.y; staging_word(lds_brick, k, 5) = rd.z;
						staging_word(lds_brick, k, 6) = scolor.x; staging_word(lds_brick, k, 7) = scolor.y; staging_word(lds_brick, k, 8) = scolor.z;
						staging_word(lds_brick, k, 9) = __uint_as_float(local_pixel);
						if (DBG) staging_word(lds_brick, k, 10) = __uint_as_float((static_cast<uint32_t>(s) << 8) | static_cast<uint32_t>(bounces));
						shadow = false;
						if (terminated) { s++; pstate = P_GEN; need_setup = false; }
						else { bounces++; ro = hitp; rd = bdir; r.n = pn; }
					}
					__builtin_amdgcn_fence(__ATOMIC_RELEASE, "wavefront");
					__builtin_amdgcn_wave_barrier();
					__builtin_amdgcn_fence(__ATOMIC_ACQUIRE, "wavefront");
					if (takes) {
						const uint32_t k = static_cast<uint32_t>(frank);
						ro = mk(staging_word(lds_brick, k, 0), staging_word(lds_brick, k, 1), staging_word(lds_brick, k, 2));
						rd = mk(staging_word(lds_brick, k, 3), staging_word(lds_brick, k, 4), staging_word(lds_brick, k, 5));
						scolor = mk(staging_word(lds_brick, k, 6), staging_word(lds_brick, k, 7), staging_word(lds_brick, k, 8));
						local_pixel = __float_as_uint(staging_word(lds_brick, k, 9));
						if (DBG) ray_key = __float_as_uint(staging_word(lds_brick, k, 10));
						shadow = true;
						pstate = P_HELPER;
						need_setup = true;
					}
				}
			}
			BM_REGION("C.generate");
			if (state == ST_NEED) {
				if (pstate == P_GEN) {
					if (s >= s_end) {
						if (HELP) {
						} else if (atomic_acc) {
							float* a = reinterpret_cast<float*>(accum + local_pixel);
							pixel_atomic_add(a + 0, acc.x); pixel_atomic_add(a + 1, acc.y); pixel_atomic_add(a + 2, acc.z); pixel_atomic_add(a + 3, acc.w);
						} else {
							pixel_store(accum + local_pixel, acc);
						}
						if (DBG && dbg && !ray_digest) {
							u32_in_global_memory* d = (u32_in_global_memory*)(dbg + static_cast<size_t>(local_pixel) * 8);
							if (sample_items) {
								if (s_end == 1) { d[0] = d0; d[1] = d1; d[2] = d2; d[3] = d3; }
								record_atomic_add((uint32_t*)(d + 4), hseg); record_atomic_add((uint32_t*)(d + 5), hsh); record_atomic_add((uint32_t*)(d + 6), next | (nsh << 16));
								record_atomic_add((uint32_t*)(d + 7), tally.index_loads - loads0);
							} else {
								d[0] = d0; d[1] = d1; d[2] = d2; d[3] = d3; d[4] = hseg; d[5] = hsh; d[6] = next | (nsh << 16);
								d[7] = tally.index_loads - loads0;
							}
						}
						state = ST_IDLE;
					} else {
						const uint32_t slot = p + static_cast<uint32_t>(fc.sample_base + s) * W * H;
						uint32_t seed = (fc.base_frame * 147565741u) * 720898027u * slot;
						primary_ray(fc, seed, xy & 0xFFFFu, xy >> 16, hitp, rd);
						pn = mk(0.f, 0.f, 0.f);
						bounces = 0;
						terminated = false;
						if (DBG) tally.paths++;
						ro = hitp;
						r.n = pn;
						shadow = false;
						need_setup = true;
					}
				}
				BM_MARK(3, t_sub);
			}
			BM_REGION("C.set-up");
			if (need_setup) {
				if (shadow) r.n = mk(0.f, 0.f, 0.f);
				if (DBG) {
					if (!(HELP && pstate == P_HELPER)) ray_key = (static_cast<uint32_t>(s) << 8) | static_cast<uint32_t>(bounces);
					ray_loads0 = tally.index_loads;
				}
				pstate = shadow ? ((HELP && pstate == P_HELPER) ? P_HELPER : P_SHD_DONE) : P_EXT_DONE;
				const int st = ray_setup<DBG, kEscape>(sc, ro, rd, r, tally, &esc, kSun && shadow ? fc.shadow_field_off : 0u);
				state = (st == ST_NEED && shadow) ? ST_CONN : st;
			}
			BM_MARK(4, t_sub);
		} else if (phase == 1) {
			BM_REGION("B.candidate");
			if (BM_PRIO) __builtin_amdgcn_s_setprio(BM_PRIO_B);
			if (BM_TIMED) { runsB++; lanesB += nB; }
#ifdef BM_SHARE_PROBE
			{
				const bool cand = state == ST_CAND;
				const uint32_t cell_id = r.p - r.field_off;
				bool dup = false;
				for (int l = 0; l < 63; ++l) {
					const uint32_t other = static_cast<uint32_t>(__builtin_amdgcn_readlane(static_cast<int>(cell_id), l));
					const bool other_cand = (__ballot(cand) >> l) & 1ull;
					dup = dup || (cand && other_cand && lane > l && other == cell_id);
				}
				const int n_dup = __popcll(__ballot(dup));
				if (__ballot(cand) != 0ull) { det[5] += 1; det[6] += n_dup ? 1 : 0; det[7] += static_cast<unsigned long long>(n_dup); }
			}
#endif
#ifdef BM_PHASE_TIMING
			uint32_t walk_trips = 0;
			if (state == ST_CAND) {
				int st = process_candidate<DBG>(sc, fc.campos, r, info, tally, lds_brick, &walk_trips);
#else
			if (state == ST_CAND) {
				int st = process_candidate<DBG>(sc, fc.campos, r, info, tally, lds_brick);
#endif
				state = (st == ST_NEED && shadow) ? ST_CONN : st;
			}
#if defined(BM_PHASE_TIMING) && !defined(BM_SHARE_PROBE)
			{
				uint32_t mx = walk_trips, sum = walk_trips;
				for (int off = 32; off > 0; off >>= 1) { const uint32_t o = __shfl_xor(mx, off, 64); mx = o > mx ? o : mx; sum += __shfl_xor(sum, off, 64); }
				if (mx) { det[5] += 1; det[6] += mx; det[7] += sum; }
			}
#endif
		} else {
			if (BM_PRIO) __builtin_amdgcn_s_setprio(BM_PRIO_A);
			const int nO = nA - nJ;
			BM_REGION("A.jump");
			if (nJ * BM_JUMP_RATIO >= nO) {
				int walkers = nA;
#pragma unroll 1
				for (int pass = 0; pass < BM_JUMP_PASSES; ++pass) {
					if (BM_TIMED) { runsJ++; lanesJ += walkers; }
					if (state == ST_JUMP || state == ST_OUTER) {
						int st;
						if (!(r.cube & kCubeNoJump)) st = field_jump<DBG, true, kEscape>(sc, r, tally, esc);
						else st = field_step<DBG>(sc, r, tally);
						state = (st == ST_NEED && shadow) ? ST_CONN : st;
					}
					if (BM_JUMP_PASSES > 1) {
						const int still = __popcll(__ballot(state == ST_JUMP) | __ballot(state == ST_OUTER));
						if (still * BM_JUMP_KEEP_DIV < walkers * BM_JUMP_KEEP_NUM || still == 0) break;
						walkers = still;
					}
				}
			} else {
				BM_REGION("A.single");
#pragma unroll 1
				for (int k = 0; k < BM_STEPS_PER_ROUND; ++k) {
					if (BM_TIMED) { runsA++; lanesA += __popcll(__ballot(state == ST_OUTER)); }
					if (state == ST_OUTER) {
						const int st = field_step<DBG>(sc, r, tally);
						state = (st == ST_NEED && shadow) ? ST_CONN : st;
					}
				}
			}
		}
		BM_REGION("loop-end");
		if (BM_TIMED) {
			const unsigned long long dt = __builtin_amdgcn_s_memtime() - t_phase;
			if (phase == 0) cycA += dt; else if (phase == 1) cycB += dt; else cycC += dt;
		}
	}

	if (DBG && counters) {
		unsigned long long v[8] = {tally.index_loads, tally.brick_tests, tally.byte_tests, tally.voxel_steps,
								   tally.extend_rays, tally.shadow_rays, tally.requests, tally.paths};
		for (int k = 0; k < 8; ++k) {
			unsigned long long t = v[k];
// ... 138 lines not shown
```

brickmap_amd/csrc/traverse.h:

```cpp
#pragma once
#include <hip/hip_runtime.h>

#include "detmath.h"
#include "device_types.h"
#include "escape.h"
#include "jump.h"
#include "steps.h"

namespace bm {

namespace {

constexpr float kPi = 3.1415926535897932f;
constexpr float kEpsilon = 0.001f;
constexpr uint32_t kLodBits = 0xFF000u;
constexpr uint32_t kUnloadedBit = 0x40000000u;
constexpr uint32_t kRequestedBit = 0x20000000u;

struct f3 {
	float x, y, z;
};
__device__ __forceinline__ f3 mk(float x, float y, float z) { return f3{x, y, z}; }
__device__ __forceinline__ f3 operator+(f3 a, f3 b) { return mk(a.x + b.x, a.y + b.y, a.z + b.z); }
__device__ __forceinline__ f3 operator-(f3 a, f3 b) { return mk(a.x - b.x, a.y - b.y, a.z - b.z); }
// ... 185 lines not shown

__device__ __forceinline__ void step_advance(RayState& r) {
	const float tx = r.tx, ty = r.ty, tz = r.tz;
	const int step_x = r.sx, step_y = r.stepy, step_z = r.stepz;
	const StepAxis m = step_choose(tx, ty, tz);
	const int step = step_pick(m, step_x, step_y, step_z);
	r.p += static_cast<uint32_t>(step);
	r.last_step = step;
	r.tx = step_add(tx, r.dx, m.x);
	r.ty = step_add(ty, r.dy, m.y);
	r.tz = step_add(tz, r.dz, m.z);
}
template <bool DBG>
__device__ __forceinline__ int field_step(const DeviceScene& sc, RayState& r, Tally& tally) {
	step_advance(r);
	const int st = field_lookup(sc, r);
	if (DBG && st != ST_NEED) tally.index_loads++;
	return st;
}

template <bool DIR = true>
__device__ __forceinline__ uint32_t jump_advance(RayState& r) {
	uint32_t cx, cy, cz;
	int axis;
	float tx = r.tx, ty = r.ty, tz = r.tz;
	const float dx = r.dx, dy = r.dy, dz = r.dz;
	const int step_x = r.sx, step_y = r.stepy, step_z = r.stepz;
	const uint32_t n = r.cube & 0xFFu;
	const float ix = DIR ? fabsf(r.d.x) : (dx > 0.f ? __builtin_amdgcn_rcpf(dx) : 0.f);
	const float iy = DIR ? fabsf(r.d.y) : (dy > 0.f ? __builtin_amdgcn_rcpf(dy) : 0.f);
	const float iz = DIR ? fabsf(r.d.z) : (dz > 0.f ? __builtin_amdgcn_rcpf(dz) : 0.f);
	dda_jump(tx, ty, tz, dx, dy, dz, ix, iy, iz, n, cx, cy, cz, axis);
	r.tx = tx; r.ty = ty; r.tz = tz;
	r.p += static_cast<uint32_t>(__mul24(static_cast<int>(cx), step_x) + __mul24(static_cast<int>(cy), step_y) + __mul24(static_cast<int>(cz), step_z));
	r.last_step = axis == 0 ? step_x : (axis == 1 ? step_y : step_z);
	return cx + cy + cz;
}
template <bool DBG, bool DIR = true, bool ESC = false>
__device__ __forceinline__ int field_jump(const DeviceScene& sc, RayState& r, Tally& tally, uint32_t esc = 0u) {
	const uint32_t cells = jump_advance<DIR>(r);
	int st = field_lookup(sc, r);
	if (ESC) st = escape_reached(r.p, esc, r.stepz) ? ST_NEED : st;
	if (DBG) tally.index_loads += cells - (st == ST_NEED ? 1u : 0u);
	return st;
}

#ifndef BM_JUMP_RATIO
#define BM_JUMP_RATIO 4
#endif
#ifndef BM_JUMP_PASSES
#define BM_JUMP_PASSES 6
#endif
#ifndef BM_JUMP_KEEP_NUM
#define BM_JUMP_KEEP_NUM 1
#endif
#ifndef BM_JUMP_KEEP_DIV
#define BM_JUMP_KEEP_DIV 4
#endif
template <bool DBG, int STEPS>
__device__ __forceinline__ int walk_round(const DeviceScene& sc, RayState& r, int state, int n_jump, int n_outer, Tally& tally, uint32_t& runs, uint32_t& lanes) {
	if (n_jump * BM_JUMP_RATIO >= n_outer) {
		int walkers = n_jump + n_outer;
#pragma unroll 1
		for (int pass = 0; pass < BM_JUMP_PASSES; ++pass) {
			if (DBG) { runs++; lanes += static_cast<uint32_t>(walkers); }
			if (state == ST_JUMP || state == ST_OUTER) {
				if (!(r.cube & kCubeNoJump)) state = field_jump<DBG, false>(sc, r, tally);
				else state = field_step<DBG>(sc, r, tally);
			}
			const int still = __popcll(__ballot(state == ST_JUMP || state == ST_OUTER));
			if (still * BM_JUMP_KEEP_DIV < walkers * BM_JUMP_KEEP_NUM || still == 0) break;
			walkers = still;
		}
	} else {
#pragma unroll 1
		for (int k = 0; k < STEPS; ++k) {
			if (DBG) { runs++; lanes += static_cast<uint32_t>(__popcll(__ballot(state == ST_OUTER))); }
			if (state == ST_OUTER) state = field_step<DBG>(sc, r, tally);
		}
	}
	return state;
}

template <bool DBG, bool ESC = false>
__device__ __forceinline__ int ray_setup(const DeviceScene& sc, f3 origin, const f3 dir, RayState& r, Tally& tally, uint32_t* esc = nullptr, uint32_t sun_plane = 0u) {
	r.hit = false;
	r.d = dir;
	float tminn = 0.f;
	const bool inside = origin.x > 0.f && origin.x < sc.grid_size_f && origin.y > 0.f && origin.y < sc.grid_size_f && origin.z > 0.f &&
						origin.z < sc.grid_height_f && (dir.x != 0.f || dir.y != 0.f || dir.z != 0.f) &&
						dir.x == dir.x && dir.y == dir.y && dir.z == dir.z;
	if (!inside) {
		const f3 t1 = (mk(0.f, 0.f, 0.f) - origin) / dir;
		const f3 t2 = (mk(sc.grid_size_f, sc.grid_size_f, sc.grid_height_f) - origin) / dir;
		const f3 tMin = mk(gmin(t1.x, t2.x), gmin(t1.y, t2.y), gmin(t1.z, t2.z));
		const f3 tMax = mk(gmax(t1.x, t2.x), gmax(t1.y, t2.y), gmax(t1.z, t2.z));
		tminn = gmax(gmax(tMin.x, 0.f), gmax(tMin.y, tMin.z));
		if (!(gmin(tMax.x, gmin(tMax.y, tMax.z)) > tminn)) return ST_NEED;
	}
	r.tminn = tminn;
	if (tminn > 0) {
		origin = origin + dir * tminn;
		const float gs = sc.grid_size_f, gh = sc.grid_height_f;
		const f3 scale = mk(1.f / (gs / gh), 1.f / (gs / gh), 1.f / (gh / gh));
		const f3 center = mk(gs / 2.f, gs / 2.f, gh / 2.f);
		const f3 d = center - origin;
		f3 to_center = mk(fabsf(d.x), fabsf(d.y), fabsf(d.z)) * scale;
		const f3 e = origin - center;
		const f3 signs = mk(static_cast<float>(isign(e.x)), static_cast<float>(isign(e.y)), static_cast<float>(isign(e.z)));
		to_center = to_center / gmax(to_center.x, gmax(to_center.y, to_center.z));
		r.n = signs * mk(truncf(to_center.x + 0.000001f), truncf(to_center.y + 0.000001f), truncf(to_center.z + 0.000001f));
		origin = origin - r.n * kEpsilon;
	}
	origin = origin / 8.f;
	r.o = origin;
	const int px = static_cast<int>(origin.x), py = static_cast<int>(origin.y), pz = static_cast<int>(origin.z);
	const int cells = sc.cells, cells_h = sc.cells_height;
	if (px < 0 || px >= cells || py < 0 || py >= cells || pz < 0 || pz >= cells_h) return ST_NEED;
	const uint32_t oct = (dir.x < 0.f ? 1u : 0u) | (dir.y < 0.f ? 2u : 0u) | (dir.z < 0.f ? 4u : 0u);
	r.field_off = sun_plane ? sun_plane : oct * sc.cf_plane;
	r.p = cell_offset(sc, r.field_off, px, py, pz);
	if (ESC) *esc = sc.escape[__umul24(oct, sc.cf_pxy) + (static_cast<uint32_t>(py + 1) << sc.cf_shift) + static_cast<uint32_t>(px + 1)];
	if (ESC) *esc = sun_plane ? sun_plane + sc.cf_plane : *esc;
	const float cbx = dir.x > 0.f ? static_cast<float>(px + 1) : static_cast<float>(px);
	const float cby = dir.y > 0.f ? static_cast<float>(py + 1) : static_cast<float>(py);
	const float cbz = dir.z > 0.f ? static_cast<float>(pz + 1) : static_cast<float>(pz);
	const int sx = isign(dir.x), sy = isign(dir.y), sz = isign(dir.z);
	r.sx = sx; r.stepy = sy << sc.cf_shift; r.stepz = __mul24(sz, static_cast<int>(sc.cf_pxy));
	const float rx = dir.x == 0.0f ? 0.0f : 1.f / dir.x;
	const float ry = dir.y == 0.0f ? 0.0f : 1.f / dir.y;
	const float rz = dir.z == 0.0f ? 0.0f : 1.f / dir.z;
	r.tx = dir.x != 0.f ? (cbx - origin.x) * rx : 1000000.f;
	r.ty = dir.y != 0.f ? (cby - origin.y) * ry : 1000000.f;
	r.tz = dir.z != 0.f ? (cbz - origin.z) * rz : 1000000.f;
	r.dx = static_cast<float>(sx) * rx; r.dy = static_cast<float>(sy) * ry; r.dz = static_cast<float>(sz) * rz;
	r.last_step = 0;
	if (DBG) tally.index_loads++;
	const int st = field_lookup(sc, r);
	return ESC && escape_reached(r.p, *esc, r.stepz) ? ST_NEED : st;
}

template <bool DBG, bool INFO = DBG, bool REQUEST = true>
__device__ __forceinline__ int process_candidate(const DeviceScene& sc, const int* campos, RayState& r, HitInfo& info, Tally& tally,
													 unsigned long long* lds_brick, uint32_t* walk_trips = nullptr) {
	int px, py, pz;
	cell_coords(sc, r, px, py, pz);
	const int sx = r.sx, sy = step_sign(r.stepy), sz = step_sign(r.stepz);
	const uint32_t sci = static_cast<uint32_t>((px >> 4) + __mul24(py >> 4, sc.sg_xy) + __mul24(pz >> 4, sc.sg_xy2));
	const uint32_t flat = (sci << 12) + static_cast<uint32_t>((px & 15) + ((py & 15) << 4) + ((pz & 15) << 8));
	const uint32_t pool = sc.pool_base[sci];
	const uint32_t index = sc.index_grid[flat];
	BrickRegs brick;
	brick.q0 = brick.q1 = brick.q2 = brick.q3 = make_uint4(0u, 0u, 0u, 0u);
	const int axis = move_axis(sc, r.last_step);
	const float new_distance = axis == 0 ? r.tx - r.dx : (axis == 1 ? r.ty - r.dy : (axis == 2 ? r.tz - r.dz : 0.f));
	r.n = mk(axis == -1 ? r.n.x : (axis == 0 ? -static_cast<float>(sx) : 0.f), axis == -1 ? r.n.y : (axis == 1 ? -static_cast<float>(sy) : 0.f),
			 axis == -1 ? r.n.z : (axis == 2 ? -static_cast<float>(sz) : 0.f));
	const int ddx = campos[0] - px, ddy = campos[1] - py, ddz = campos[2] - pz;
	const int lod2 = __mul24(ddx, ddx) + __mul24(ddy, ddy) + __mul24(ddz, ddz);
	float sub_distance = 0.f;
	if (INFO) info.brick_id = px + py * sc.cells + pz * sc.cells * sc.cells;
	if (lod2 > sc.lod_distance_8x8x8) {
		r.distance = new_distance * 8.f + r.tminn;
		if (INFO) { info.level = 0; info.sub_id = 0; }
		r.hit = true;
		return ST_NEED;
	} else if (lod2 > sc.lod_distance_2x2x2) {
		if (DBG) tally.byte_tests++;
		int sub = 0;
		const f3 o2 = (r.o + r.d * new_distance) * 2.f - r.n * 0.2f * kEpsilon;
		if (intersect_grid<2, DBG>(o2, r.d, sx, sy, sz, r.dx, r.dy, r.dz, r.n, sub_distance, brick, (index & kLodBits) >> 12, sub, tally)) {
			r.distance = new_distance * 8.f + sub_distance * 4.f + r.tminn;
			if (INFO) { info.level = 1; info.sub_id = sub; }
			r.hit = true;
			return ST_NEED;
		}
	} else if (index & kLoadedBit) {
		if (DBG) tally.brick_tests++;
		int sub = 0;
		const f3 o8 = (r.o + r.d * new_distance) * 8.f - r.n * kEpsilon;
		const uint4* bq = reinterpret_cast<const uint4*>(sc.brick_arena + (static_cast<size_t>(pool + (index & kIndexBits)) << 4));
		if (!BM_LDS_DMA) { brick.q0 = bq[0]; brick.q1 = bq[1]; brick.q2 = bq[2]; brick.q3 = bq[3]; }
		if (intersect_grid<8, DBG>(o8, r.d, sx, sy, sz, r.dx, r.dy, r.dz, r.n, sub_distance, brick, 0u, sub, tally, lds_brick, walk_trips, reinterpret_cast<const uint32_t*>(bq))) {
			r.distance = new_distance * 8.f + sub_distance + r.tminn;
			if (INFO) { info.level = 2; info.sub_id = sub; }
			r.hit = true;
			return ST_NEED;
		}
	} else if (index & kUnloadedBit) {
		const uint32_t old = REQUEST ? atomicOr(&sc.index_grid[flat], kRequestedBit) : kRequestedBit;
		if (!(old & kRequestedBit)) {
			const uint32_t load_index = atomicAdd(sc.load_queue_count, 1u);
			if (load_index < sc.queue_cap) {
				int* q = sc.load_queue + 3 * static_cast<size_t>(load_index);
				q[0] = px; q[1] = py; q[2] = pz;
				if (DBG) tally.requests++;
			} else {
				atomicAnd(&sc.index_grid[flat], ~kRequestedBit);
			}
		}
		r.distance = new_distance * 8.f + r.tminn;
		if (INFO) { info.level = 3; info.sub_id = 0; }
		r.hit = true;
		return ST_NEED;
	}
	return ST_OUTER;
}

__device__ __forceinline__ float fast_div(float a, float b) { return a * __builtin_amdgcn_rcpf(b); }
__device__ __forceinline__ float fast_sqrt(float a) { return __builtin_amdgcn_sqrtf(a); }
__device__ __forceinline__ float fast_exp(float a) { return __expf(a); }
struct SkyView {
	f3 Fex;
	float cosViewSun;
};
__device__ __forceinline__ SkyView sky_view(const FrameConstants& fc, f3 viewDir) {
	SkyView o;
	o.cosViewSun = dot(viewDir, ld3(fc.sun_direction));
	const float cosUpView = dot(mk(0.f, 0.f, 1.f), viewDir);
	const float zenith = gmax(0.0f, cosUpView);
	const float inv_zenith = __builtin_amdgcn_rcpf(zenith);
	const float rayleighLen = 8.4E3f * inv_zenith;
// ... 121 lines not shown
```

brickmap_amd/host.py:

```python
import ctypes as C
import math
import os
from dataclasses import dataclass, field, replace

import numpy as np

from . import _lib
from ._lib import (BM_EDIT_BOX, BM_EDIT_CLEAR, BM_EDIT_SET, BM_EDIT_SPHERE, BM_REGION_REPLACE, bm_region, BM_QUERY_LOD, BM_QUERY_NO_REQUESTS, BM_VOLUME_ANY, BM_VOXELS_DEVICE, BM_VOXELS_HOST, bm_camera, bm_counters, bm_edit, bm_frame_params,
                   bm_scene_info, check)


FLYTHROUGH_VIEWS = (
    ((512.0, 512.0, 300.0), (-61863.5, -0.501796)),
    ((840.254, 832.446, 1169.88), (-61864.4, -0.429796)),
    ((2227.83, 774.886, 204.955), (-61863.9, 0.0622036)),
    ((3326.19, 2055.72, 44.7995), (-61864.2, -0.981796)),
    ((7134.6, 1262.44, 5531.79), (-61865.2, -0.501796)),
    ((11298.6, 3113.03, 598.019), (-61866.3, -0.141796)),
    ((10921.4, 4774.14, 267.808), (-61859.4, 0.0142036)),
    ((9961.29, 4508.12, 189.59), (-61857.2, -0.261796)),
    ((10835.3, 4160.83, 359.992), (-61857.2, -0.261796)),
)


# ... 489 lines not shown
                check(self._L.bm_scene_load_voxels(self.gpuScene, C.c_void_p(volume.data_ptr()), volume.numel(), BM_VOXELS_DEVICE, C.c_void_p(target.cuda_stream)))
                return self
            volume = volume.numpy()
        check(self._L.bm_scene_load_voxels(self.gpuScene, C.c_void_p(volume.ctypes.data), volume.size, BM_VOXELS_HOST, None))
        return self

    @classmethod
    def from_voxels(cls, volume, device=0):
        grid_size, grid_height = volume_dims(volume)
        return cls(grid_size, grid_height, device=device).load_voxels(volume)

    def voxels(self):
        out = np.zeros((self.grid_height, self.grid_size, self.grid_size), np.uint8)
        n = C.c_size_t(0)
        check(self._L.bm_scene_host_voxels(self.gpuScene, out.ctypes.data, out.size, C.byref(n)))
        return out.view(np.bool_)

    def last_load_ms(self):
        a, b, c = C.c_float(0), C.c_float(0), C.c_float(0)
        check(self._L.bm_scene_last_load_ms(self.gpuScene, C.byref(a), C.byref(b), C.byref(c)))
        return float(a.value), float(b.value), float(c.value)

    def _stream(self, stream):
        if stream is None:
            import torch
            stream = torch.cuda.current_stream(self.device).cuda_stream
        return C.c_void_p(stream)

    def edit(self, edits, stream=None):
        arr, count = _edit_array(edits)
        check(self._L.bm_scene_edit(self.gpuScene, count, arr, self._stream(stream)))
        return self

    def fill_box(self, lo, hi, stream=None):
        return self.edit([edit_box(BM_EDIT_SET, lo, hi)], stream)

    def clear_box(self, lo, hi, stream=None):
        return self.edit([edit_box(BM_EDIT_CLEAR, lo, hi)], stream)

    def fill_sphere(self, center, radius, stream=None):
        return self.edit([edit_sphere(BM_EDIT_SET, center, radius)], stream)

    def carve_sphere(self, center, radius, stream=None):
        return self.edit([edit_sphere(BM_EDIT_CLEAR, center, radius)], stream)

    def set_voxels(self, coords, values, stream=None):
        if hasattr(coords, "detach"):
            coords = coords.detach().cpu().numpy()
        xyz = np.ascontiguousarray(np.asarray(coords).reshape(-1, 3), dtype=np.int32)
        if hasattr(values, "detach"):
            values = values.detach().cpu().numpy()
        v = np.asarray(values)
        v = np.full(len(xyz), 1 if v.item() else 0, np.uint8) if v.ndim == 0 else np.ascontiguousarray(v != 0, dtype=np.uint8)
        assert len(v) == len(xyz), "values: a scalar or one per voxel"
        check(self._L.bm_scene_set_voxels(self.gpuScene, len(xyz), xyz.ctypes.data, v.ctypes.data, self._stream(stream)))
        return self

    def _cube_field(self, fn):
        n = C.c_size_t(0)
        check(fn(self.gpuScene, None, 0, C.byref(n)))
        out = np.zeros(n.value, np.uint8)
        check(fn(self.gpuScene, out.ctypes.data, out.size, C.byref(n)))
        cx, cz = self.grid_size // 8 + 2, self.grid_height // 8 + 2
        return out.reshape(8, cz, cx, cx)

    def device_cube_field(self):
        return self._cube_field(self._L.bm_scene_device_cube_field)

    def host_cube_field(self):
        return self._cube_field(self._L.bm_scene_host_cube_field)

    def sun_plane(self):
        n = C.c_size_t(0)
        plan = (C.c_int32 * 12)()
        check(self._L.bm_scene_sun_plane(self.gpuScene, None, 0, C.byref(n), plan))
        names = ("valid", "octant", "dom", "m1", "m2", "lo1", "hi1", "lo2", "hi2", "clear", "rise", "bins")
        plan = dict(zip(names, (int(v) for v in plan)))
        if n.value == 0:
            return None, plan
        out = np.zeros(n.value, np.uint8)
        check(self._L.bm_scene_sun_plane(self.gpuScene, out.ctypes.data, out.size, C.byref(n), None))
        c = self.grid_size // 8 + 2
        return out.reshape(-1, c, c), plan

    def sun_plane_stats(self):
        builds, ms = C.c_uint64(0), C.c_float(0)
        check(self._L.bm_scene_sun_plane_stats(self.gpuScene, C.byref(builds), C.byref(ms)))
        return int(builds.value), float(ms.value)

    def escape_table(self):
        n = C.c_size_t(0)
        check(self._L.bm_scene_escape_table(self.gpuScene, None, 0, C.byref(n)))
        out = np.zeros(n.value, np.int32)
        check(self._L.bm_scene_escape_table(self.gpuScene, out.ctypes.data, out.size, C.byref(n)))
        c = self.grid_size // 8
        return out.reshape(8, c, c)

    def last_edit_ms(self):
        a, b = C.c_float(0), C.c_float(0)
        check(self._L.bm_scene_last_edit_ms(self.gpuScene, C.byref(a), C.byref(b)))
        return float(a.value), float(b.value)

    def _volume_stream(self, tensor, stream):
        import torch
        if tensor.device.index != self.device:
            raise ValueError(f"a tensor on cuda:{self.device} (the scene's GPU) or on the CPU expected, got {tensor.device}")
        current = torch.cuda.current_stream(tensor.device)
        target = current if stream is None else torch.cuda.ExternalStream(int(stream), device=tensor.device)
        if target.cuda_stream != current.cuda_stream:
            target.wait_stream(current)
        return current, target

    def write_region(self, lo, volume, op="replace", stream=None):
        r, ptr, cuda = region_of(lo, volume)
        if min(volume.shape) == 0:
            return self
        if cuda:
            _, target = self._volume_stream(volume, stream)
            check(self._L.bm_scene_write_region(self.gpuScene, C.byref(r), _region_op(op), C.c_void_p(ptr), BM_VOXELS_DEVICE, C.c_void_p(target.cuda_stream)))
        else:
            check(self._L.bm_scene_write_region(self.gpuScene, C.byref(r), _region_op(op), C.c_void_p(ptr), BM_VOXELS_HOST, self._stream(stream)))
        return self

    def read_region(self, lo, hi, out=None, device=False, stream=None):
        shape = tuple(int(h) - int(l) for l, h in zip(lo, hi))[::-1]
        if min(shape) < 0:
            raise ValueError(f"read_region: hi < lo ({lo} ... {hi})")
        result = out
        if out is None:
            if device:
                import torch
                out = result = torch.empty(shape, dtype=torch.uint8, device=f"cuda:{self.device}")
            else:
                out = np.zeros(shape, np.uint8)
                result = out.view(np.bool_)
        elif tuple(out.shape) != shape:
            raise ValueError(f"read_region: out of shape {shape} expected, got {tuple(out.shape)}")
        r, ptr, cuda = region_of(lo, out, "out")
        if min(shape) == 0:
            return result
        if cuda:
            current, target = self._volume_stream(out, stream)
            check(self._L.bm_scene_read_region(self.gpuScene, C.byref(r), C.c_void_p(ptr), BM_VOXELS_DEVICE, C.c_void_p(target.cuda_stream)))
            if target.cuda_stream != current.cuda_stream:
                current.wait_stream(target)
        else:
            check(self._L.bm_scene_read_region(self.gpuScene, C.byref(r), C.c_void_p(ptr), BM_VOXELS_HOST, None))
        return result

    def last_region_ms(self):
        t = [C.c_float(0) for _ in range(4)]
        check(self._L.bm_scene_last_region_ms(self.gpuScene, *[C.byref(v) for v in t]))
        return tuple(float(v.value) for v in t)

    def cast_rays_raw(self, n, rays_ptr, hits_ptr, flags=0, lod_origin=None, stream=None):
        lo = None if lod_origin is None else (C.c_float * 3)(*[float(v) for v in lod_origin])
        check(self._L.bm_scene_cast_rays(self.gpuScene, int(n), C.c_void_p(rays_ptr), C.c_void_p(hits_ptr), int(flags), lo, self._stream(stream)))

    def cast_rays(self, origins, directions=None, tmax=None, lod_origin=None, request=True, stream=None):
        import torch
        flags = (BM_QUERY_LOD if lod_origin is not None else 0) | (0 if request else BM_QUERY_NO_REQUESTS)
        dev = origins.device if isinstance(origins, torch.Tensor) else torch.device("cuda", self.device)
        current = torch.cuda.current_stream(dev)
        target = current if stream is None else torch.cuda.ExternalStream(int(stream), device=dev)
        other = target.cuda_stream != current.cuda_stream
        if other:
# ... 432 lines not shown
```

include/brickmap.h:

```cpp
#ifndef BRICKMAP_H
#define BRICKMAP_H

#include <stddef.h>
#include <stdint.h>

#ifdef __cplusplus
extern "C" {
#endif

#define BM_API __attribute__((visibility("default")))

#define BM_EINVAL 10001
#define BM_ESTATE 10002

#define BM_BRICK_INDEX_BITS 0x00000FFFu
#define BM_BRICK_LOD_BITS 0x000FF000u
#define BM_BRICK_REQUESTED_BIT 0x20000000u
#define BM_BRICK_UNLOADED_BIT 0x40000000u
#define BM_BRICK_LOADED_BIT 0x80000000u

#define BM_FLAG_PRIMARY_ONLY 1u
#define BM_FLAG_COUNTERS 2u
#define BM_FLAG_SAMPLE_ITEMS 4u

// ... 21 lines not shown
	uint32_t flags;
	int32_t band_rows, shard_rank, shard_count;
	float sun_position[2];
} bm_frame_params;

typedef struct bm_scene_info {
	int32_t grid_size, grid_height;
	int32_t supergrid_xy, supergrid_z, supercells;
	int32_t queue_capacity;
	int32_t lod_distance_8x8x8, lod_distance_2x2x2;
	int32_t generated, on_device;
	uint64_t total_bricks;
	uint64_t resident_bricks;
	uint64_t index_bytes, brick_bytes;
	uint64_t pool_bytes;
	uint64_t cube_field_bytes;
	uint64_t arena_growths;
	uint64_t arena_copy_growths;
	int32_t arena_virtual;
	int32_t failed;
	uint64_t stream_batches;
	uint64_t stream_host_ns;
	uint64_t escape_bytes;
	uint64_t sun_plane_bytes;
} bm_scene_info;

#define BM_EDIT_SET 1
#define BM_EDIT_CLEAR 2
#define BM_EDIT_BOX 1
#define BM_EDIT_SPHERE 2
typedef struct bm_edit {
	int32_t op;
	int32_t shape;
	int32_t lo[3];
	int32_t hi[3];
	int32_t center[3];
	int32_t radius;
} bm_edit;

typedef struct bm_counters {
	uint64_t index_loads, brick_tests, byte_tests, voxel_steps, extend_rays, shadow_rays, requests, paths;
} bm_counters;

typedef struct bm_sched_stats {
	uint64_t step_runs, step_lanes;
	uint64_t candidate_runs, candidate_lanes;
	uint64_t shade_runs, shade_lanes;
	uint64_t connect_runs, connect_lanes;
	uint64_t step_cycles, candidate_cycles, shade_cycles;
	uint64_t drain_cycles;
	uint64_t total_cycles;
	uint64_t jump_runs, jump_lanes;
	uint64_t waves;
} bm_sched_stats;

BM_API const char* bm_last_error_string(void);
BM_API int bm_device_count(int* count);
BM_API int bm_device_name(int device, char* buf, size_t buflen, int* compute_units);

BM_API int bm_scene_create(int device, int grid_size, int grid_height, bm_scene** out);
BM_API void bm_scene_destroy(bm_scene* scene);
BM_API int bm_scene_set_lod(bm_scene* scene, int lod_distance_8x8x8, int lod_distance_2x2x2);
BM_API int bm_scene_set_queue_capacity(bm_scene* scene, int capacity);
BM_API int bm_scene_set_streaming_mode(bm_scene* scene, int overlapped);
BM_API int bm_scene_generate(bm_scene* scene, int threads);
BM_API int bm_scene_generate_supercell(bm_scene* scene, int sx, int sy, int sz);
BM_API int bm_scene_preload_all(bm_scene* scene);
BM_API int bm_scene_reset_residency(bm_scene* scene);
BM_API int bm_scene_process_load_queue(bm_scene* scene, uint32_t* serviced);
BM_API int bm_scene_dump(bm_scene* scene, const char* path);
BM_API int bm_scene_get_info(bm_scene* scene, bm_scene_info* info);
BM_API int bm_scene_host_supercell(bm_scene* scene, int supercell, uint32_t* indices4096, uint32_t* brick_count,
                                   uint32_t* bricks, uint32_t brick_capacity);
BM_API int bm_scene_device_indices(bm_scene* scene, int supercell, uint32_t* indices4096);
BM_API int bm_scene_device_brick(bm_scene* scene, int supercell, uint32_t device_slot, uint32_t* brick16);
BM_API int bm_scene_column_heights(bm_scene* scene, int sx, int sy, float* heights128x128);

BM_API int bm_scene_edit(bm_scene* scene, int count, const bm_edit* edits, void* hip_stream);
BM_API int bm_scene_set_voxels(bm_scene* scene, int n, const int32_t* xyz, const uint8_t* values, void* hip_stream);
BM_API int bm_scene_device_cube_field(bm_scene* scene, uint8_t* dst, size_t capacity, size_t* bytes);
BM_API int bm_scene_host_cube_field(bm_scene* scene, uint8_t* dst, size_t capacity, size_t* bytes);
BM_API int bm_scene_escape_table(bm_scene* scene, int32_t* dst, size_t capacity, size_t* count);
BM_API int bm_scene_sun_plane(bm_scene* scene, uint8_t* dst, size_t capacity, size_t* bytes, int32_t* plan12);
BM_API int bm_scene_sun_plane_stats(bm_scene* scene, uint64_t* builds, float* last_build_ms);
BM_API int bm_scene_last_edit_ms(bm_scene* scene, float* scatter_ms, float* field_ms);

#define BM_VOXELS_HOST   0
#define BM_VOXELS_DEVICE 1
BM_API int bm_scene_load_voxels(bm_scene* scene, const uint8_t* voxels, size_t bytes, int where, void* hip_stream);
BM_API int bm_scene_host_voxels(bm_scene* scene, uint8_t* dst, size_t capacity, size_t* bytes);
BM_API int bm_scene_last_load_ms(bm_scene* scene, float* pack_ms, float* field_ms, float* mirror_ms);

typedef struct bm_region {
	int32_t lo[3], hi[3];
	int64_t row_pitch;
	int64_t slice_pitch;
} bm_region;
#define BM_REGION_REPLACE 0
BM_API int bm_scene_write_region(bm_scene* scene, const bm_region* region, int op, const uint8_t* voxels, int where, void* hip_stream);
BM_API int bm_scene_read_region(bm_scene* scene, const bm_region* region, uint8_t* voxels, int where, void* hip_stream);
BM_API int bm_scene_last_region_ms(bm_scene* scene, float* pack_ms, float* copy_ms, float* scatter_ms, float* field_ms);

typedef struct bm_ray {
	float origin[3];
	float direction[3];
	float tmax;
	uint32_t reserved;
} bm_ray;
typedef struct bm_ray_hit {
	float distance;
	float normal[3];
	int32_t voxel[3];
	int32_t level;
} bm_ray_hit;
#define BM_QUERY_LOD         1u
#define BM_QUERY_NO_REQUESTS 2u
BM_API int bm_scene_cast_rays(bm_scene* scene, int64_t n, const bm_ray* rays_dev, bm_ray_hit* hits_dev, uint32_t flags,
                              const float lod_origin[3], void* hip_stream);
BM_API int bm_camera_pixel_rays(const bm_camera* camera, int width, int height, int64_t n, const float* px, const float* py, bm_ray* out);

BM_API int bm_camera_pixel_rays_device(bm_scene* scene, const bm_camera* camera, int width, int height, bm_ray* rays_dev, void* hip_stream);

typedef struct bm_denoise_params {
	int32_t width, height;
	int32_t iterations;
	float sigma_l;
	uint32_t flags;
	uint32_t reserved;
} bm_denoise_params;
BM_API int bm_denoise_workspace_bytes(int width, int height, size_t* bytes);
BM_API int bm_denoise(bm_scene* scene, const bm_denoise_params* params, const float* accum_dev, const bm_ray_hit* hits_dev, float* out_dev,
                      void* workspace_dev, size_t workspace_bytes, void* hip_stream);
BM_API int bm_debug_denoise_times(bm_scene* scene, const bm_denoise_params* params, const float* accum_dev, const bm_ray_hit* hits_dev, float* out_dev,
                                  void* workspace_dev, size_t workspace_bytes, void* hip_stream, float* kernel_ms);
BM_API int bm_host_denoise(const bm_denoise_params* params, const float* accum, const bm_ray_hit* hits, float* out);

typedef struct bm_reproject_params {
	int32_t width, height;
	float max_history;
	uint32_t flags;
	uint32_t reserved;
} bm_reproject_params;
BM_API int bm_history_bytes(int width, int height, size_t* bytes);
BM_API int bm_reproject(bm_scene* scene, const bm_reproject_params* params, const bm_camera* camera, const bm_camera* camera_prev,
                        const float* accum_dev, const bm_ray_hit* hits_dev, const void* history_prev_dev, void* history_out_dev, void* hip_stream);
BM_API int bm_host_reproject(const bm_reproject_params* params, const bm_camera* camera, const bm_camera* camera_prev, const float* accum,
                             const bm_ray_hit* hits, const void* history_prev, void* history_out);

typedef struct bm_volume {
	int32_t shape;
	int32_t lo[3], hi[3];
	int32_t center[3];
	int32_t radius;
	uint32_t reserved;
} bm_volume;
typedef struct bm_volume_result {
	uint64_t solid;
	int32_t lo[3], hi[3];
	uint32_t unresolved;
	uint32_t status;
} bm_volume_result;
#define BM_VOLUME_ANY 1u
BM_API int bm_scene_query_volumes(bm_scene* scene, int64_t n, const bm_volume* volumes_dev, bm_volume_result* results_dev, uint32_t flags,
                                  void* hip_stream);

BM_API int bm_host_column_heights(int grid_size, int grid_height, int sx, int sy, float* heights128x128);
// ... 106 lines not shown
```

Before: 12730.

## Add sun shadow-height table to terminate shadow rays early in dark columns

Adds a per-column shadow height table, built alongside the sun field by sweeping slabs along the sun direction from the top of solid columns. Shadow rays whose start cell lies below that height are marked as hit at setup and skip traversal. The table is rebuilt incrementally over the touched xy box after edits, and the sun build can now refresh only the shadow part without rebuilding the field. This adds build kernels, an extra escape-table slice and one extra comparison in ray setup, and a conservative margin is needed to keep the shadowing correct.

```diff
diff --git a/brickmap_amd/_lib.py b/brickmap_amd/_lib.py
--- a/brickmap_amd/_lib.py
+++ b/brickmap_amd/_lib.py
@@ -147,6 +147,7 @@
     "bm_scene_host_cube_field": (_i, [_vp, _vp, C.c_size_t, C.POINTER(C.c_size_t)]),
     "bm_scene_escape_table": (_i, [_vp, _vp, C.c_size_t, C.POINTER(C.c_size_t)]),
     "bm_scene_sun_plane": (_i, [_vp, _vp, C.c_size_t, C.POINTER(C.c_size_t), _vp]),
+    "bm_scene_shadow_heights": (_i, [_vp, _vp, C.c_size_t, C.POINTER(C.c_size_t), C.POINTER(C.c_uint64), _vp]),
     "bm_scene_sun_plane_stats": (_i, [_vp, C.POINTER(C.c_uint64), C.POINTER(C.c_float)]),
     "bm_scene_last_edit_ms": (_i, [_vp, C.POINTER(C.c_float), C.POINTER(C.c_float)]),
     "bm_scene_load_voxels": (_i, [_vp, _vp, C.c_size_t, _i, _vp]),
diff --git a/brickmap_amd/csrc/capi.cpp b/brickmap_amd/csrc/capi.cpp
--- a/brickmap_amd/csrc/capi.cpp
+++ b/brickmap_amd/csrc/capi.cpp
@@ -127,6 +127,7 @@
 int bm_scene_host_cube_field(bm_scene* scene, uint8_t* dst, size_t capacity, size_t* bytes) { BM_NEED(scene); return scene->impl.host_cube_field(dst, capacity, bytes); }
 int bm_scene_escape_table(bm_scene* scene, int32_t* dst, size_t capacity, size_t* count) { BM_NEED(scene); return scene->impl.escape_table(dst, capacity, count); }
 int bm_scene_sun_plane(bm_scene* scene, uint8_t* dst, size_t capacity, size_t* bytes, int32_t* plan12) { BM_NEED(scene); return scene->impl.sun_plane(dst, capacity, bytes, plan12); }
+int bm_scene_shadow_heights(bm_scene* scene, uint32_t* dst, size_t capacity, size_t* count, uint64_t* bytes, int32_t* plan4) { BM_NEED(scene); return scene->impl.shadow_heights(dst, capacity, count, bytes, plan4); }
 int bm_scene_sun_plane_stats(bm_scene* scene, uint64_t* builds, float* last_build_ms) { BM_NEED(scene); return scene->impl.sun_plane_stats(builds, last_build_ms); }
 int bm_scene_last_edit_ms(bm_scene* scene, float* scatter_ms, float* field_ms) { BM_NEED(scene); return scene->impl.last_edit_ms(scatter_ms, field_ms); }
 
diff --git a/brickmap_amd/csrc/kernels.h b/brickmap_amd/csrc/kernels.h
--- a/brickmap_amd/csrc/kernels.h
+++ b/brickmap_amd/csrc/kernels.h
@@ -3,6 +3,7 @@
 
 #include "device_types.h"
 #include "reproject.h"
+#include "shadowheight.h"
 #include "sunfield.h"
 
 namespace bm {
@@ -48,13 +49,17 @@
 
 struct SunBuild {
 	SunPlan plan;
+	ShadowPlan shadow;
+	int fx0, fx1, fy0, fy1;
 	int cells, cells_height, sg_xy, sg_xy2;
 	int nd, n1, n2;
 	int cf_shift;
 	uint32_t cf_pxy, cf_plane;
 };
 size_t sun_build_tmp_bytes(const SunBuild& u);
-void launch_sun_build(const uint32_t* index_grid, const int32_t* cols, const uint32_t* escape, uint8_t* field, uint8_t* tmp, const SunBuild& u, hipStream_t stream);
+size_t shadow_build_tmp_bytes(const SunBuild& u);
+void launch_sun_build(const uint32_t* index_grid, const uint32_t* pool_base, const uint32_t* arena, const int32_t* cols, uint32_t* escape, uint8_t* field, uint8_t* tmp,
+					  uint8_t* tmp_shadow, const SunBuild& u, bool with_field, hipStream_t stream);
 
 struct LoadDims {
 	uint32_t grid_size;
diff --git a/brickmap_amd/csrc/scene.cpp b/brickmap_amd/csrc/scene.cpp
--- a/brickmap_amd/csrc/scene.cpp
+++ b/brickmap_amd/csrc/scene.cpp
@@ -155,6 +155,8 @@
 	use_ring(0);
 	snapshot_pending_ = false;
 	preloaded_ = preloaded;
+	shadow_dirty_ = true;
+	shadow_full_valid_ = false;
 	staging_busy_ = false;
 	failed_ = false;
 	stream_batches_ = stream_host_ns_ = 0;
@@ -276,6 +278,8 @@
 	}
 	if (!sun_plane_) { if (int e = d_cube_field_.alloc(l.plane * 8)) return e; }
 	sun_built_ = false;
+	shadow_full_valid_ = false;
+	shadow_zero_ = true;
 	sun_dirty_ = true;
 	BM_HIP(hipMemset(d_cube_field_, 255, d_cube_field_.bytes()));
 	view_.cf_shift = l.shift;
@@ -283,7 +287,7 @@
 	view_.cf_plane = static_cast<uint32_t>(l.plane);
 	division_magic(view_.cf_pxy, &view_.cf_magic, &view_.cf_magic_shift);
 	view_.cube_field = d_cube_field_;
-	if (int e = d_escape_.alloc(escape_entries(view_.cf_pxy) * sizeof(uint32_t))) return e;
+	if (int e = d_escape_.alloc((escape_entries(view_.cf_pxy) + (BM_SHADOWHEIGHT != 0 ? view_.cf_pxy : 0u)) * sizeof(uint32_t))) return e;
 	BM_HIP(hipMemset(d_escape_, 0, d_escape_.bytes()));
 	if (int e = d_escape_cols_.alloc(escape_columns_bytes(world.dims.cells))) return e;
 	view_.escape = d_escape_;
@@ -747,7 +751,7 @@
 	out->brick_bytes = on_device_ ? arena_.capacity() * 64 : 0;
 	out->pool_bytes = on_device_ ? arena_.pool_bricks() * 64 : 0;
 	out->cube_field_bytes = on_device_ ? 8 * static_cast<uint64_t>(view_.cf_plane) : 0;
-	out->escape_bytes = on_device_ ? d_escape_.bytes() : 0;
+	out->escape_bytes = on_device_ ? escape_entries(view_.cf_pxy) * sizeof(uint32_t) : 0;
 	out->sun_plane_bytes = on_device_ && sun_plane_ ? static_cast<uint64_t>(view_.cf_plane) + d_sun_tmp_.bytes() : 0;
 	out->arena_growths = arena_.growths();
 	out->arena_copy_growths = arena_.copy_growths();
@@ -841,6 +845,11 @@
 	for (int j = 0; j < kCellsPerSupercell; ++j) {
 		if (!touched[j]) continue;
 		const uint32_t ow = old_words[j], nw = c.indices[j];
+		{
+			const int gx = sx * kSupercell + (j & 15), gy = sy * kSupercell + ((j >> 4) & 15);
+			b.touch_lo[0] = std::min(b.touch_lo[0], gx); b.touch_hi[0] = std::max(b.touch_hi[0], gx);
+			b.touch_lo[1] = std::min(b.touch_lo[1], gy); b.touch_hi[1] = std::max(b.touch_hi[1], gy);
+		}
 		const uint16_t ods = ow ? old_dev[ow & BM_BRICK_INDEX_BITS] : kNoDeviceSlot;
 		if (ods != kNoDeviceSlot) {
 			if (nw) dev[nw & BM_BRICK_INDEX_BITS] = ods;
@@ -934,6 +943,8 @@
 							load_stream_);
 		BM_HIP(hipGetLastError());
 		BM_HIP(hipEventRecord(times[1], load_stream_));
+		shadow_dirty_ = true;
+		for (int k = 0; k < 2; ++k) { shadow_box_[k] = std::min(shadow_box_[k], b.touch_lo[k]); shadow_box_[2 + k] = std::max(shadow_box_[2 + k], b.touch_hi[k]); }
 		if (field) {
 			launch_field_update(d_index_grid_, d_cube_field_, d_cf_tmp_, fu, load_stream_);
 			BM_HIP(hipGetLastError());
@@ -1189,11 +1200,18 @@
 	if (!plan.valid) return 0;
 	const float key[4] = {fc.cone_dir[0], fc.cone_dir[1], fc.cone_dir[2], fc.cone_extent};
 	*usable = true;
-	if (sun_built_ && !sun_dirty_ && std::memcmp(key, sun_key_, sizeof key) == 0) return 0;
+	const bool stands = sun_built_ && !sun_dirty_ && std::memcmp(key, sun_key_, sizeof key) == 0;
+	if (stands && !(BM_SHADOWHEIGHT != 0 && shadow_dirty_)) return 0;
 	const WorldDims& d = world.dims;
 	const int n[3] = {d.cells, d.cells, d.cells_height};
 	SunBuild u{};
 	u.plan = plan;
+	u.shadow = BM_SHADOWHEIGHT != 0 && preloaded_ ? shadow_plan(fc.cone_dir, fc.cone_extent) : ShadowPlan{};
+	if (stands && !u.shadow.valid && shadow_zero_) {
+		shadow_dirty_ = false;
+		shadow_plan_ = u.shadow;
+		return 0;
+	}
 	u.cells = d.cells; u.cells_height = d.cells_height;
 	u.sg_xy = d.supergrid_xy; u.sg_xy2 = d.supergrid_xy * d.supergrid_xy;
 	u.nd = n[plan.dom]; u.n1 = n[plan.m1]; u.n2 = n[plan.m2];
@@ -1204,9 +1222,20 @@
 		BM_HIP(hipStreamSynchronize(load_stream_));
 		if (d_sun_tmp_.reserve(sun_build_tmp_bytes(u)) != 0) { (void)hipGetLastError(); set_error(""); return 0; }
 	}
+	if (u.shadow.valid && shadow_build_tmp_bytes(u) > d_shadow_tmp_.bytes()) {
+		BM_HIP(hipStreamSynchronize(load_stream_));
+		shadow_full_valid_ = false;
+		if (d_shadow_tmp_.reserve(shadow_build_tmp_bytes(u)) != 0) { (void)hipGetLastError(); set_error(""); return 0; }
+	}
+	if (!shadow_full_valid_) { u.fx0 = u.fy0 = 0; u.fx1 = u.fy1 = d.cells; }
+	else {
+		u.fx0 = std::max(0, shadow_box_[0]); u.fy0 = std::max(0, shadow_box_[1]);
+		u.fx1 = std::min(d.cells, shadow_box_[2] + 1); u.fy1 = std::min(d.cells, shadow_box_[3] + 1);
+		if (u.fx1 <= u.fx0 || u.fy1 <= u.fy0) u.fx0 = u.fx1 = u.fy0 = u.fy1 = 0;
+	}
 	if (int e = order_load_stream_behind_frames()) return e;
 	BM_HIP(hipEventRecord(ev_sun_time_[0], load_stream_));
-	launch_sun_build(d_index_grid_, d_escape_cols_, d_escape_, d_cube_field_, d_sun_tmp_, u, load_stream_);
+	launch_sun_build(d_index_grid_, d_pool_base_, arena_.base(), d_escape_cols_, d_escape_, d_cube_field_, d_sun_tmp_, d_shadow_tmp_, u, !stands, load_stream_);
 	BM_HIP(hipGetLastError());
 	BM_HIP(hipEventRecord(ev_sun_time_[1], load_stream_));
 	BM_HIP(hipEventRecord(ev_upload_, load_stream_));
@@ -1215,7 +1244,14 @@
 	sun_plan_ = plan;
 	sun_built_ = true;
 	sun_dirty_ = false;
-	sun_builds_++;
+	shadow_dirty_ = false;
+	shadow_plan_ = u.shadow;
+	shadow_zero_ = !u.shadow.valid;
+	if (u.shadow.valid) {
+		shadow_full_valid_ = true;
+		shadow_box_[0] = shadow_box_[1] = 1 << 30; shadow_box_[2] = shadow_box_[3] = -1;
+	}
+	if (!stands) sun_builds_++;
 	*usable = true;
 	return 0;
 }
@@ -1236,6 +1272,30 @@
 	BM_HIP(hipSetDevice(device_));
 	BM_HIP(hipDeviceSynchronize());
 	BM_HIP(hipMemcpy2D(dst, X, d_cube_field_ + 8 * static_cast<size_t>(view_.cf_plane), static_cast<size_t>(1) << view_.cf_shift, X, X * Z, hipMemcpyDeviceToHost));
+	return 0;
+}
+
+int Scene::shadow_heights(uint32_t* dst, size_t capacity, size_t* count, uint64_t* bytes, int32_t* plan4) {
+	if (int e = require_on_device()) return e;
+	const WorldDims& d = world.dims;
+	const bool have = BM_SHADOWHEIGHT != 0 && sun_plane_ && sun_built_;
+	const size_t need = have ? static_cast<size_t>(d.cells) * d.cells : 0;
+	if (count) *count = need;
+	if (bytes) *bytes = BM_SHADOWHEIGHT != 0 && on_device_ ? static_cast<uint64_t>(view_.cf_pxy) * sizeof(uint32_t) + d_shadow_tmp_.bytes() : 0;
+	if (plan4) {
+		const ShadowPlan p = have ? shadow_plan_ : ShadowPlan{};
+		const int32_t v[4] = {p.valid, p.sun.rise, p.rise_hi, kSunHeightUnit};
+		std::memcpy(plan4, v, sizeof v);
+	}
+	if (!dst || !have) return 0;
+	if (capacity < need) { set_error("shadow heights buffer too small"); return BM_EINVAL; }
+	BM_HIP(hipSetDevice(device_));
+	BM_HIP(hipDeviceSynchronize());
+	std::vector<uint32_t> slice(view_.cf_pxy);
+	BM_HIP(hipMemcpy(slice.data(), d_escape_ + escape_entries(view_.cf_pxy), slice.size() * sizeof(uint32_t), hipMemcpyDeviceToHost));
+	for (int y = 0; y < d.cells; ++y)
+		for (int x = 0; x < d.cells; ++x)
+			dst[static_cast<size_t>(y) * d.cells + x] = slice[escape_index(0, view_.cf_shift, view_.cf_pxy, x, y)];
 	return 0;
 }
 
diff --git a/brickmap_amd/csrc/scene.h b/brickmap_amd/csrc/scene.h
--- a/brickmap_amd/csrc/scene.h
+++ b/brickmap_amd/csrc/scene.h
@@ -40,6 +40,7 @@
 	int last_edit_ms(float* scatter_ms, float* field_ms);
 	int sun_plane(uint8_t* dst, size_t capacity, size_t* bytes, int32_t* plan12);
 	int sun_plane_stats(uint64_t* builds, float* last_build_ms);
+	int shadow_heights(uint32_t* dst, size_t capacity, size_t* count, uint64_t* bytes, int32_t* plan4);
 	int write_region(const bm_region* region, int op, const uint8_t* voxels, int where, hipStream_t stream);
 	int read_region(const bm_region* region, uint8_t* voxels, int where, hipStream_t stream);
 	int last_region_ms(float* pack_ms, float* copy_ms, float* scatter_ms, float* field_ms);
@@ -85,6 +86,7 @@
 		std::vector<Brick> bricks;
 		std::vector<PoolMove> moves;
 		int box_lo[3] = {1 << 30, 1 << 30, 1 << 30}, box_hi[3] = {-1, -1, -1};
+		int touch_lo[2] = {1 << 30, 1 << 30}, touch_hi[2] = {-1, -1};
 	};
 	int wait_edit_staging();
 	int stage_touched(int sci, const std::vector<uint32_t>& old_words, const uint8_t* touched, DeviceBatch& b);
@@ -132,8 +134,13 @@
 	bool sun_plane_ = false, sun_built_ = false, sun_dirty_ = true;
 	float sun_key_[4] = {0.f, 0.f, 0.f, 0.f};
 	SunPlan sun_plan_{};
+	bool shadow_dirty_ = true;
+	bool shadow_zero_ = true;
+	bool shadow_full_valid_ = false;
+	int shadow_box_[4] = {1 << 30, 1 << 30, -1, -1};
+	ShadowPlan shadow_plan_{};
 	uint64_t sun_builds_ = 0;
-	DeviceBuffer<uint8_t> d_sun_tmp_;
+	DeviceBuffer<uint8_t> d_sun_tmp_, d_shadow_tmp_;
 	Event ev_sun_time_[2];
 	DeviceBuffer<int> d_load_queue_[2];
 	DeviceBuffer<uint32_t> d_load_count_[2];
diff --git a/brickmap_amd/csrc/shadowheight.h b/brickmap_amd/csrc/shadowheight.h
--- /dev/null
+++ b/brickmap_amd/csrc/shadowheight.h
@@ -0,0 +1,81 @@
+#pragma once
+#include <cstdint>
+
+#include "sunfield.h"
+
+#ifndef BM_SHADOWHEIGHT
+#define BM_SHADOWHEIGHT 1
+#endif
+#ifndef BM_SHADOWHEIGHT_XCD
+#define BM_SHADOWHEIGHT_XCD 0
+#endif
+
+namespace bm {
+
+struct ShadowPlan {
+	SunPlan sun;
+	int valid;
+	int rise_hi;
+};
+
+#ifndef BM_SHADOWHEIGHT_LOOSE
+#define BM_SHADOWHEIGHT_LOOSE 0
+#endif
+
+BM_JHD ShadowPlan shadow_plan(const float dir[3], float extent) {
+	ShadowPlan sp{};
+	sp.sun = sun_plan(dir, extent);
+	if (!sp.sun.valid || !sp.sun.clear) return sp;
+	const double e = extent;
+	double s = 1.0 - (1.0 - e) * (1.0 - e);
+	s = s > 0.0 ? s : 0.0;
+	{
+		double q = s > 0.0 ? 1.0 : 0.0;
+		for (int i = 0; i < 60 && q > 0.0; ++i) q = 0.5 * (q + s / q);
+		s = q;
+	}
+	const double r = s * 1.05 + 2e-3;
+	const double az = dir[2] < 0.0f ? -static_cast<double>(dir[2]) : dir[2], ad = dir[sp.sun.dom] < 0.0f ? -static_cast<double>(dir[sp.sun.dom]) : dir[sp.sun.dom];
+	const double shi = (az + r) / (ad - r);
+	const double h = shi * kSunHeightUnit + 0.5;
+	sp.rise_hi = static_cast<int>(h) + 1;
+#if BM_SHADOWHEIGHT_LOOSE == 1
+	sp.rise_hi = sp.sun.rise;
+#endif
+	sp.valid = 1;
+	return sp;
+}
+
+constexpr int kShadowMargin =
+#if BM_SHADOWHEIGHT_LOOSE == 2
+	-kSunHeightUnit;
+#else
+	kSunHeightMargin;
+#endif
+
+template <class Next>
+BM_JHD int shadow_next_least(int w, int glo, int ghi, Next next) {
+	int least = 1 << 30;
+	for (int g = glo; g <= ghi; ++g) {
+		const int n = next(w + g / kSunBins, g % kSunBins);
+		least = n < least ? n : least;
+	}
+	return least;
+}
+template <class Next>
+BM_JHD int shadow_face_value(const ShadowPlan& p, int w, int b, int full, Next next) {
+	const int n = shadow_next_least(w, b + p.sun.lo1, b + p.sun.hi1, next) - p.rise_hi;
+	return n > full ? n : full;
+}
+template <class Next>
+BM_JHD int shadow_dark_cells(const ShadowPlan& p, int w, int nz, Next next) {
+	const int t = shadow_next_least(w, 0, kSunBins - 1 + p.sun.hi1, next) - p.rise_hi - kShadowMargin;
+	const int z = t > 0 ? (t - 1) / kSunHeightUnit : 0;
+	return z < nz ? z : nz;
+}
+
+BM_JHD uint32_t shadow_entry(uint32_t sun_plane_offset, uint32_t cf_pxy, int dark_cells) {
+	return dark_cells > 0 ? sun_plane_offset + static_cast<uint32_t>(dark_cells + 1) * cf_pxy : 0u;
+}
+
+}
diff --git a/brickmap_amd/csrc/shadowheight_host.h b/brickmap_amd/csrc/shadowheight_host.h
--- /dev/null
+++ b/brickmap_amd/csrc/shadowheight_host.h
@@ -0,0 +1,34 @@
+#pragma once
+#include <cstdint>
+#include <vector>
+
+#include "shadowheight.h"
+
+namespace bm {
+
+inline void shadow_heights_host(const ShadowPlan& p, const int n[3], const std::vector<uint8_t>& full, std::vector<int>& zd) {
+	zd.assign(static_cast<size_t>(n[0]) * n[1], 0);
+	if (!p.valid) return;
+	const SunPlan& s = p.sun;
+	const int B = kSunBins, nd = n[s.dom], n1 = n[s.m1], nz = n[2];
+	auto column = [&](int ud, int w) { int c[3] = {0, 0, 0}; c[s.dom] = sun_coord(s, s.dom, nd, ud); c[s.m1] = sun_coord(s, s.m1, n1, w); return static_cast<size_t>(c[1]) * n[0] + c[0]; };
+	std::vector<int> top(zd.size(), 0);
+	for (int y = 0; y < n[1]; ++y)
+		for (int x = 0; x < n[0]; ++x) {
+			int z = 0;
+			while (z < nz && full[(static_cast<size_t>(z) * n[1] + y) * n[0] + x]) ++z;
+			top[static_cast<size_t>(y) * n[0] + x] = z * kSunHeightUnit;
+		}
+	std::vector<int> sn(static_cast<size_t>(n1) * B, 0), sc(sn.size());
+	for (int ud = nd - 1; ud >= 0; --ud) {
+		auto next = [&](int w, int b) { return w < n1 ? sn[static_cast<size_t>(w) * B + b] : 0; };
+		for (int w = 0; w < n1; ++w) {
+			const size_t col = column(ud, w);
+			zd[col] = shadow_dark_cells(p, w, nz, next);
+			for (int b = 0; b < B; ++b) sc[static_cast<size_t>(w) * B + b] = shadow_face_value(p, w, b, top[col], next);
+		}
+		sn.swap(sc);
+	}
+}
+
+}
diff --git a/brickmap_amd/csrc/sunfield.hip b/brickmap_amd/csrc/sunfield.hip
--- a/brickmap_amd/csrc/sunfield.hip
+++ b/brickmap_amd/csrc/sunfield.hip
@@ -15,6 +15,17 @@
 	int32_t* clear[2];
 	uint8_t* face[2];
 };
+struct ShadowTmp {
+	int32_t* full;
+	int32_t* shade[2];
+};
+__host__ __device__ inline ShadowTmp shadow_tmp(uint8_t* tmp, const SunBuild& u) {
+	ShadowTmp t;
+	t.full = reinterpret_cast<int32_t*>(tmp);
+	t.shade[0] = t.full + static_cast<size_t>(u.cells) * u.cells;
+	t.shade[1] = t.shade[0] + static_cast<size_t>(u.n1) * kSunBins;
+	return t;
+}
 __host__ __device__ inline SunTmp sun_tmp(uint8_t* tmp, const SunBuild& u) {
 	const size_t n1 = static_cast<size_t>(u.n1), n2 = static_cast<size_t>(u.n2);
 	SunTmp t;
@@ -45,8 +56,27 @@
 	((g_i32*)stamped)[t] = sun_first_stamped(1 << 20, quadrant_threshold(escape, u, x, y));
 }
 
-__global__ void sun_clear_slab(const int32_t* __restrict__ cols, const uint32_t* __restrict__ escape, int32_t* __restrict__ stamped, const int32_t* __restrict__ cn,
-							   int32_t* __restrict__ cc, const SunBuild u, const int ud) {
+__global__ void shadow_full_tops(const uint32_t* __restrict__ index_grid, const uint32_t* __restrict__ pool_base, const uint32_t* __restrict__ arena, int32_t* __restrict__ full,
+								 const SunBuild u) {
+	const uint32_t t = blockIdx.x * blockDim.x + threadIdx.x;
+	const uint32_t nx = static_cast<uint32_t>(u.fx1 - u.fx0), ny = static_cast<uint32_t>(u.fy1 - u.fy0);
+	if (t >= nx * ny) return;
+	const int x = u.fx0 + static_cast<int>(t % nx), y = u.fy0 + static_cast<int>(t / nx);
+	int z = 0;
+	for (; z < u.cells_height; ++z) {
+		const uint32_t word = ld32(index_grid, index_word_at(u.sg_xy, u.sg_xy2, x, y, z));
+		if (!(word & kLoadedBit) || (word & 0xFF000u) != 0xFF000u) break;
+		const size_t first = brick_first_word(ld32(pool_base, supercell_of(u.sg_xy, u.sg_xy2, x, y, z)), word);
+		uint32_t all = 0xFFFFFFFFu;
+		for (int k = 0; k < 4; ++k) { const u32x4 v = ld128(arena, static_cast<int64_t>((first + 4 * k) * sizeof(uint32_t))); all &= v.x & v.y & v.z & v.w; }
+		if (all != 0xFFFFFFFFu) break;
+	}
+	((g_i32*)full)[static_cast<size_t>(y) * u.cells + x] = z * kSunHeightUnit;
+}
+
+template <bool CLEAR, bool SHADE>
+__global__ void sun_clear_slab(const int32_t* __restrict__ cols, uint32_t* __restrict__ escape, int32_t* __restrict__ stamped, const int32_t* __restrict__ cn,
+							   int32_t* __restrict__ cc, const int32_t* __restrict__ full, const int32_t* __restrict__ sn, int32_t* __restrict__ sc, const SunBuild u, const int ud) {
 	const SunPlan& p = u.plan;
 	const int n1 = u.n1;
 	const uint32_t t = blockIdx.x * blockDim.x + threadIdx.x;
@@ -59,10 +89,18 @@
 		return (ldi32(cols, static_cast<size_t>(y) * u.cells + x) + 1) * kSunHeightUnit;
 	};
 	auto next = [&](int ww, int bb) { return ww < n1 ? ldi32(cn, static_cast<size_t>(ww) * kSunBins + bb) : 0; };
-	((g_i32*)cc)[t] = sun_clear_face_value(p, w, b, height, next);
-	if (b == 0) {
+	if (CLEAR) {
+		((g_i32*)cc)[t] = sun_clear_face_value(p, w, b, height, next);
+		if (b == 0) {
+			int x, y; column(w, x, y);
+			((g_i32*)stamped)[static_cast<size_t>(y) * u.cells + x] = sun_first_stamped(sun_clear_cell(p, w, height, next), quadrant_threshold(escape, u, x, y));
+		}
+	}
+	if (SHADE) {
+		auto shade_next = [&](int ww, int bb) { return ww < n1 ? ldi32(sn, static_cast<size_t>(ww) * kSunBins + bb) : 0; };
 		int x, y; column(w, x, y);
-		((g_i32*)stamped)[static_cast<size_t>(y) * u.cells + x] = sun_first_stamped(sun_clear_cell(p, w, height, next), quadrant_threshold(escape, u, x, y));
+		((g_i32*)sc)[t] = shadow_face_value(u.shadow, w, b, ldi32(full, static_cast<size_t>(y) * u.cells + x), shade_next);
+		if (b == 0) st32(escape, escape_index(8, u.cf_shift, u.cf_pxy, x, y), shadow_entry(8u * u.cf_plane, u.cf_pxy, shadow_dark_cells(u.shadow, w, u.cells_height, shade_next)));
 	}
 }
 
@@ -106,20 +144,40 @@
 	const size_t n1 = static_cast<size_t>(u.n1), n2 = static_cast<size_t>(u.n2);
 	return (static_cast<size_t>(u.cells) * u.cells + 2 * n1 * kSunBins) * sizeof(int32_t) + 2 * n1 * n2 * kSunBins * kSunBins;
 }
+size_t shadow_build_tmp_bytes(const SunBuild& u) {
+	return (static_cast<size_t>(u.cells) * u.cells + 2 * static_cast<size_t>(u.n1) * kSunBins) * sizeof(int32_t);
+}
 
-void launch_sun_build(const uint32_t* index_grid, const int32_t* cols, const uint32_t* escape, uint8_t* field, uint8_t* tmp, const SunBuild& u, hipStream_t stream) {
+void launch_sun_build(const uint32_t* index_grid, const uint32_t* pool_base, const uint32_t* arena, const int32_t* cols, uint32_t* escape, uint8_t* field, uint8_t* tmp,
+					  uint8_t* tmp_shadow, const SunBuild& u, bool with_field, hipStream_t stream) {
 	const SunPlan& p = u.plan;
 	const SunTmp t = sun_tmp(tmp, u);
+	const ShadowTmp h = shadow_tmp(tmp_shadow, u);
 	const int nd = u.nd;
 	const uint32_t columns = static_cast<uint32_t>(u.cells) * static_cast<uint32_t>(u.cells), clear_lanes = static_cast<uint32_t>(u.n1) * kSunBins;
 	const size_t face_bytes = static_cast<size_t>(t.face[1] - t.face[0]);
 	const uint32_t face_lanes = static_cast<uint32_t>(face_bytes);
-	(void)hipMemsetAsync(t.clear[0], 0, clear_lanes * sizeof(int32_t), stream);
-	(void)hipMemsetAsync(t.face[0], 0, face_bytes, stream);
-	if (!p.clear) hipLaunchKernelGGL(sun_stamp_quadrant, dim3((columns + 63) / 64), dim3(64), 0, stream, escape, t.stamped, u);
+	const bool shade = BM_SHADOWHEIGHT != 0 && u.shadow.valid != 0;
+	if (with_field) {
+		(void)hipMemsetAsync(t.clear[0], 0, clear_lanes * sizeof(int32_t), stream);
+		(void)hipMemsetAsync(t.face[0], 0, face_bytes, stream);
+		if (!p.clear) hipLaunchKernelGGL(sun_stamp_quadrant, dim3((columns + 63) / 64), dim3(64), 0, stream, escape, t.stamped, u);
+	}
+	if (BM_SHADOWHEIGHT != 0) {
+		if (shade) {
+			(void)hipMemsetAsync(h.shade[0], 0, clear_lanes * sizeof(int32_t), stream);
+			const uint32_t scanned = static_cast<uint32_t>(u.fx1 - u.fx0) * static_cast<uint32_t>(u.fy1 - u.fy0);
+			if (scanned) hipLaunchKernelGGL(shadow_full_tops, dim3((scanned + 63) / 64), dim3(64), 0, stream, index_grid, pool_base, arena, h.full, u);
+		} else {
+			(void)hipMemsetAsync(escape + escape_entries(u.cf_pxy), 0, static_cast<size_t>(u.cf_pxy) * sizeof(uint32_t), stream);
+		}
+	}
+	const dim3 cg((clear_lanes + 63) / 64), cb(64);
 	for (int ud = nd - 1, k = 0; ud >= 0; --ud, k ^= 1) {
-		if (p.clear) hipLaunchKernelGGL(sun_clear_slab, dim3((clear_lanes + 63) / 64), dim3(64), 0, stream, cols, escape, t.stamped, t.clear[k], t.clear[k ^ 1], u, ud);
-		hipLaunchKernelGGL(sun_field_slab, dim3((face_lanes + 255) / 256), dim3(256), 0, stream, index_grid, t.stamped, t.face[k], t.face[k ^ 1], field, u, ud);
+		if (with_field && p.clear && shade) hipLaunchKernelGGL((sun_clear_slab<true, true>), cg, cb, 0, stream, cols, escape, t.stamped, t.clear[k], t.clear[k ^ 1], h.full, h.shade[k], h.shade[k ^ 1], u, ud);
+		else if (with_field && p.clear) hipLaunchKernelGGL((sun_clear_slab<true, false>), cg, cb, 0, stream, cols, escape, t.stamped, t.clear[k], t.clear[k ^ 1], h.full, h.shade[k], h.shade[k ^ 1], u, ud);
+		else if (shade) hipLaunchKernelGGL((sun_clear_slab<false, true>), cg, cb, 0, stream, cols, escape, t.stamped, t.clear[k], t.clear[k ^ 1], h.full, h.shade[k], h.shade[k ^ 1], u, ud);
+		if (with_field) hipLaunchKernelGGL(sun_field_slab, dim3((face_lanes + 255) / 256), dim3(256), 0, stream, index_grid, t.stamped, t.face[k], t.face[k ^ 1], field, u, ud);
 	}
 }
 
diff --git a/brickmap_amd/csrc/trace.hip b/brickmap_amd/csrc/trace.hip
--- a/brickmap_amd/csrc/trace.hip
+++ b/brickmap_amd/csrc/trace.hip
@@ -105,6 +105,7 @@
 	RayState r;
 	constexpr bool kEscape = BM_ESCAPE != 0 && !DBG && (BM_ESCAPE_XCD != 0 || !XCD);
 	constexpr bool kSun = BM_SUNFIELD != 0 && kEscape && (BM_SUNFIELD_XCD != 0 || !XCD);
+	constexpr bool kShade = BM_SHADOWHEIGHT != 0 && kSun && !DBG && (BM_SHADOWHEIGHT_XCD != 0 || !XCD);
 	uint32_t esc = 0;
 	r.hit = false;
 	r.n = mk(0.f, 0.f, 0.f);
@@ -501,7 +502,7 @@
 					ray_loads0 = tally.index_loads;
 				}
 				pstate = shadow ? ((HELP && pstate == P_HELPER) ? P_HELPER : P_SHD_DONE) : P_EXT_DONE;
-				const int st = ray_setup<DBG, kEscape>(sc, ro, rd, r, tally, &esc, kSun && shadow ? fc.shadow_field_off : 0u);
+				const int st = ray_setup<DBG, kEscape, kShade>(sc, ro, rd, r, tally, &esc, kSun && shadow ? fc.shadow_field_off : 0u);
 				state = (st == ST_NEED && shadow) ? ST_CONN : st;
 			}
 			BM_MARK(4, t_sub);
diff --git a/brickmap_amd/csrc/traverse.h b/brickmap_amd/csrc/traverse.h
--- a/brickmap_amd/csrc/traverse.h
+++ b/brickmap_amd/csrc/traverse.h
@@ -291,7 +291,7 @@
 	return state;
 }
 
-template <bool DBG, bool ESC = false>
+template <bool DBG, bool ESC = false, bool SHADE = false>
 __device__ __forceinline__ int ray_setup(const DeviceScene& sc, f3 origin, const f3 dir, RayState& r, Tally& tally, uint32_t* esc = nullptr, uint32_t sun_plane = 0u) {
 	r.hit = false;
 	r.d = dir;
@@ -329,7 +329,8 @@
 	const uint32_t oct = (dir.x < 0.f ? 1u : 0u) | (dir.y < 0.f ? 2u : 0u) | (dir.z < 0.f ? 4u : 0u);
 	r.field_off = sun_plane ? sun_plane : oct * sc.cf_plane;
 	r.p = cell_offset(sc, r.field_off, px, py, pz);
-	if (ESC) *esc = sc.escape[__umul24(oct, sc.cf_pxy) + (static_cast<uint32_t>(py + 1) << sc.cf_shift) + static_cast<uint32_t>(px + 1)];
+	if (ESC) *esc = sc.escape[__umul24(SHADE && sun_plane ? 8u : oct, sc.cf_pxy) + (static_cast<uint32_t>(py + 1) << sc.cf_shift) + static_cast<uint32_t>(px + 1)];
+	const bool dark = ESC && SHADE && sun_plane != 0u && r.p < *esc;
 	if (ESC) *esc = sun_plane ? sun_plane + sc.cf_plane : *esc;
 	const float cbx = dir.x > 0.f ? static_cast<float>(px + 1) : static_cast<float>(px);
 	const float cby = dir.y > 0.f ? static_cast<float>(py + 1) : static_cast<float>(py);
@@ -346,7 +347,8 @@
 	r.last_step = 0;
 	if (DBG) tally.index_loads++;
 	const int st = field_lookup(sc, r);
-	return ESC && escape_reached(r.p, *esc, r.stepz) ? ST_NEED : st;
+	if (SHADE) r.hit = dark;
+	return ESC && (escape_reached(r.p, *esc, r.stepz) || dark) ? ST_NEED : st;
 }
 
 template <bool DBG, bool INFO = DBG, bool REQUEST = true>
diff --git a/brickmap_amd/host.py b/brickmap_amd/host.py
--- a/brickmap_amd/host.py
+++ b/brickmap_amd/host.py
@@ -595,6 +595,18 @@
         check(self._L.bm_scene_sun_plane(self.gpuScene, out.ctypes.data, out.size, C.byref(n), None))
         c = self.grid_size // 8 + 2
         return out.reshape(-1, c, c), plan
+
+    def shadow_heights(self):
+        n, nbytes = C.c_size_t(0), C.c_uint64(0)
+        plan = (C.c_int32 * 4)()
+        check(self._L.bm_scene_shadow_heights(self.gpuScene, None, 0, C.byref(n), C.byref(nbytes), plan))
+        plan = dict(zip(("valid", "rise", "rise_hi", "unit"), (int(v) for v in plan)))
+        if n.value == 0:
+            return None, plan, int(nbytes.value)
+        out = np.zeros(n.value, np.uint32)
+        check(self._L.bm_scene_shadow_heights(self.gpuScene, out.ctypes.data, out.size, C.byref(n), None, None))
+        c = self.grid_size // 8
+        return out.reshape(c, c), plan, int(nbytes.value)
 
     def sun_plane_stats(self):
         builds, ms = C.c_uint64(0), C.c_float(0)
diff --git a/include/brickmap.h b/include/brickmap.h
--- a/include/brickmap.h
+++ b/include/brickmap.h
@@ -127,6 +127,7 @@
 BM_API int bm_scene_host_cube_field(bm_scene* scene, uint8_t* dst, size_t capacity, size_t* bytes);
 BM_API int bm_scene_escape_table(bm_scene* scene, int32_t* dst, size_t capacity, size_t* count);
 BM_API int bm_scene_sun_plane(bm_scene* scene, uint8_t* dst, size_t capacity, size_t* bytes, int32_t* plan12);
+BM_API int bm_scene_shadow_heights(bm_scene* scene, uint32_t* dst, size_t capacity, size_t* count, uint64_t* bytes, int32_t* plan4);
 BM_API int bm_scene_sun_plane_stats(bm_scene* scene, uint64_t* builds, float* last_build_ms);
 BM_API int bm_scene_last_edit_ms(bm_scene* scene, float* scatter_ms, float* field_ms);
 
```

Result: faster. 14020, median of 6 (+10.1%).
